# argumentcomputer/lurk-beta

Hardware: AMD Instinct MI355X
Metric: MSM Mscalar-mul/s (Pallas Pedersen commitment, bases+scalars resident in HBM) (higher is better)
Workload: dtype u32x8 (255-bit Montgomery, integer VALU)

## Files before the change

lurk_beta_amd/csrc/curve29.cuh:

```cuda
#pragma once
#include "curve.cuh"
#include "field29.cuh"

#ifndef LURK_ACC_Y3_ROW
#define LURK_ACC_Y3_ROW 1
#endif
#ifndef LURK_ACC_AFFINE_FIRST
#define LURK_ACC_AFFINE_FIRST 1
#endif
#ifndef LURK_F29_RARE_ATTR
#define LURK_F29_RARE_ATTR __attribute__((noinline))
#endif

namespace lurk {

template <class P>
LURK_HD F29<P> f29_carry_signed(const int32_t* t) {
    F29<P> r;
    int32_t c = 0;
#pragma unroll
    for (int i = 0; i < 8; i++) {
        int32_t x = t[i] + c;
        r.l[i] = (uint32_t)x & F29_MASK;
        c = x >> 29;
    }
    r.l[8] = (uint32_t)(t[8] + c);
    return r;
}


template <class P>
LURK_HD F29<P> f29_reduce_pasta(const F29<P>& v) {
    const uint32_t k = v.l[8] >> 22;
    const uint32_t km1 = k ? k - 1 : 0;
    int32_t t[9];
    uint64_t c = 0;
#pragma unroll
    for (int i = 0; i < 5; i++) {
        c += (uint64_t)km1 * f29_mod<P>(i);
        t[i] = (int32_t)v.l[i] - (int32_t)((uint32_t)c & F29_MASK);
        c >>= 29;
    }
    t[5] = (int32_t)v.l[5] - (int32_t)(uint32_t)c;
    t[6] = (int32_t)v.l[6];
    t[7] = (int32_t)v.l[7];
    t[8] = (int32_t)(v.l[8] & ((1u << 22) - 1u)) + (k ? (int32_t)(1u << 22) : 0);
    return f29_carry_signed<P>(t);
}
template <class P>
LURK_HD F29<P> f29_reduce_general(const F29<P>& v) {
    constexpr uint32_t D = (P::mod(7) >> 8) + 1u;
    static_assert(D > (1u << 21) && D <= (1u << 22), "f29_reduce_general: the modulus must have 253 or 254 bits");
    constexpr uint64_t mu = ((uint64_t)1 << 53) / D;
    F29_ASSERT(v.l[8] < (1u << 31), "f29_reduce: top limb >= 2^31");
    const uint32_t q = (uint32_t)(((uint64_t)v.l[8] * mu) >> 53);
    int32_t t[9];
    uint64_t c = 0;
#pragma unroll
    for (int i = 0; i < 8; i++) {
        c += (uint64_t)q * f29_mod<P>(i);
        t[i] = (int32_t)v.l[i] - (int32_t)((uint32_t)c & F29_MASK);
        c >>= 29;
    }
    c += (uint64_t)q * f29_mod<P>(8);
    t[8] = (int32_t)v.l[8] - (int32_t)(uint32_t)c;
    const F29<P> r = f29_carry_signed<P>(t);
    F29_ASSERT(r.l[8] < (1u << 24), "f29_reduce: result not below 2^256");
    return r;
}
template <class P>
LURK_HD F29<P> f29_reduce(const F29<P>& v) {
    if constexpr (f29_pasta_shape<P>()) return f29_reduce_pasta<P>(v);
    else return f29_reduce_general<P>(v);
}

template <class P>
struct Xyzz29 {
    F29<P> x, y, zz, zzz;
};

template <class P>
LURK_HD Xyzz<P> xyzz29_to_xyzz(const Xyzz29<P>& a, bool is_identity) {
    if (is_identity) return xyzz_identity<P>();
    Xyzz<P> r;
    r.x = f29_to_mont256<P>(a.x);
    r.y = f29_to_mont256<P>(a.y);
    r.zz = f29_to_mont256<P>(a.zz);
    r.zzz = f29_to_mont256<P>(a.zzz);
    return r;
}
template <class P>
LURK_HD void xyzz29_from_xyzz(const Xyzz<P>& a, Xyzz29<P>& r, bool& is_identity) {
    is_identity = xyzz_is_identity<P>(a);
    r.x = f29_from_mont256<P>(a.x);
    r.y = f29_from_mont256<P>(a.y);
    r.zz = f29_from_mont256<P>(a.zz);
    r.zzz = f29_from_mont256<P>(a.zzz);
}

template <class P>
LURK_HD uint32_t f29_multiple_candidate(const F29<P>& v) {
    if constexpr (f29_pasta_shape<P>()) return v.l[0];
    else return (v.l[0] * ((0u - f29_inv<P>()) & F29_MASK)) & F29_MASK;
}
template <class P>
LURK_HD bool f29_maybe_multiple_of_p(const F29<P>& v) {
    return f29_multiple_candidate<P>(v) < (f29_pasta_shape<P>() ? 128u : 256u);
}
template <class P>
LURK_HD bool f29_is_multiple_of_p(const F29<P>& v) {
    const uint32_t k = f29_multiple_candidate<P>(v);
    uint64_t c = 0;
    bool eq = true;
#pragma unroll
    for (int i = 0; i < 8; i++) {
        c += (uint64_t)k * f29_mod<P>(i);
        eq = eq && (v.l[i] == ((uint32_t)c & F29_MASK));
        c >>= 29;
    }
    c += (uint64_t)k * f29_mod<P>(8);
    return eq && (uint64_t)v.l[8] == c;
}

template <class P>
LURK_HD LURK_F29_RARE_ATTR Xyzz29<P> xyzz29_double_affine(F29<P> qx, F29<P> qy_signed) {
    const F29<P> u = f29_dbl<P>(qy_signed);
    const F29<P> v = f29_mul<P>(u, u);
    const F29<P> w = f29_mul30<P>(u, v);
    const F29<P> s = f29_mul30<P>(qx, v);
    const F29<P> xx = f29_sqr30<P>(qx);
    const F29<P> m = f29_carry<P>(f29_add<P>(f29_dbl<P>(xx), xx));
    const F29<P> m2 = f29_sqr30<P>(m);
    Xyzz29<P> r;
    r.x = f29_reduce<P>(f29_carry<P>(f29_sub<P>(m2, f29_dbl<P>(s))));
    const F29<P> t1 = f29_mul<P>(m, f29_sub<P>(s, r.x));
    const F29<P> t2 = f29_mul30<P>(w, qy_signed);
    r.y = f29_reduce<P>(f29_carry<P>(f29_sub<P>(t1, t2)));
    r.zz = v;
    r.zzz = w;
    return r;
}

template <class P, bool ACC_AFFINE = false>
LURK_HD void xyzz29_madd(Xyzz29<P>& acc, bool& acc_id, const Affine<P>& q, bool negate) {
    if (affine_is_identity<P>(q)) return;
    const F29<P> qx = f29_from_mont256<P>(q.x);
    const F29<P> qy = f29_from_mont256<P>(q.y);
    if (acc_id) {
        acc.x = qx;
        acc.y = negate ? f29_reduce<P>(f29_carry<P>(f29_sub<P>(f29_zero<P>(), qy))) : qy;
        Fe<P> one = fe_one<P>();
        acc.zz = f29_from_mont256<P>(one);
        acc.zzz = acc.zz;
        acc_id = false;
        return;
    }
    F29_ASSERT_LIMBS(acc.x, 29, "acc.x"); F29_ASSERT_TOP(acc.x, 27, "acc.x");
    F29_ASSERT_LIMBS(acc.y, 29, "acc.y"); F29_ASSERT_TOP(acc.y, 27, "acc.y");
    F29_ASSERT_LIMBS(acc.zz, 29, "acc.zz"); F29_ASSERT_TOP(acc.zz, 27, "acc.zz");
    F29_ASSERT_LIMBS(acc.zzz, 29, "acc.zzz"); F29_ASSERT_TOP(acc.zzz, 27, "acc.zzz");
    const F29<P> u2 = ACC_AFFINE ? qx : f29_mul30<P>(qx, acc.zz);
    const F29<P> s2 = ACC_AFFINE ? qy : f29_mul30<P>(qy, acc.zzz);
    const F29<P> p = f29_carry<P>(f29_sub<P>(u2, acc.x));
    F29<P> r;
#pragma unroll
    for (int i = 0; i < 9; i++) {
        F29_ASSERT(f29_bias<P>(i) >= acc.y.l[i], "madd: Y1 limb above the bias");
        r.l[i] = s2.l[i] + (negate ? acc.y.l[i] : f29_bias<P>(i) - acc.y.l[i]);
    }
    r = f29_carry<P>(r);
    if (f29_maybe_multiple_of_p<P>(p) && f29_is_multiple_of_p<P>(p)) {
        if (f29_maybe_multiple_of_p<P>(r) && f29_is_multiple_of_p<P>(r)) {
            const F29<P> qys = negate ? f29_reduce<P>(f29_carry<P>(f29_sub<P>(f29_zero<P>(), qy))) : qy;
            acc = xyzz29_double_affine<P>(qx, qys);
        } else {
            acc_id = true;
        }
        return;
    }
    const F29<P> pp = f29_sqr30<P>(p);
    const F29<P> ppp = f29_mul30<P>(p, pp);
    const F29<P> qq = f29_mul30<P>(acc.x, pp);
    const F29<P> r2 = f29_sqr30<P>(r);
    F29<P> x3 = f29_sub<P>(f29_sub<P>(r2, ppp), f29_dbl<P>(qq));
    x3 = f29_reduce<P>(f29_carry<P>(x3));
    F29<P> d;
#pragma unroll
    for (int i = 0; i < 9; i++) {
        F29_ASSERT(f29_bias<P>(i) >= qq.l[i] && f29_bias<P>(i) >= x3.l[i], "madd: Q / X3 limb above the bias");
        d.l[i] = negate ? x3.l[i] + (f29_bias<P>(i) - qq.l[i]) : qq.l[i] + (f29_bias<P>(i) - x3.l[i]);
    }
#if LURK_ACC_Y3_ROW
    Dot29<P> row;
    dot29_init<P>(row);
    dot29_mac<P>(row, r, f29_carry<P>(d));
    dot29_mac<P>(row, f29_carry<P>(f29_sub<P>(f29_zero<P>(), acc.y)), ppp);
    F29<P> y3 = f29_reduce<P>(dot29_finish2<P>(row));
#else
    const F29<P> t1 = f29_mul<P>(r, d);
    const F29<P> t2 = f29_mul30<P>(acc.y, ppp);
    F29<P> y3 = f29_reduce<P>(f29_carry<P>(f29_sub<P>(t1, t2)));
#endif
    acc.x = x3;
    acc.y = y3;
    if (ACC_AFFINE) {
        acc.zz = f29_reduce<P>(pp);
        acc.zzz = f29_reduce<P>(ppp);
    } else {
        acc.zz = f29_mul30<P>(acc.zz, pp);
        acc.zzz = f29_mul30<P>(acc.zzz, ppp);
    }
}

template <class P>
LURK_HD Xyzz29<P> xyzz29_dbl(const Xyzz29<P>& a) {
    const F29<P> u = f29_dbl<P>(a.y);
    const F29<P> v = f29_mul<P>(u, u);
    const F29<P> w = f29_mul30<P>(u, v);
    const F29<P> s = f29_mul30<P>(a.x, v);
    const F29<P> xx = f29_sqr30<P>(a.x);
    const F29<P> m = f29_carry<P>(f29_add<P>(f29_dbl<P>(xx), xx));
    const F29<P> m2 = f29_sqr30<P>(m);
    Xyzz29<P> r;
    r.x = f29_reduce<P>(f29_carry<P>(f29_sub<P>(m2, f29_dbl<P>(s))));
    const F29<P> t1 = f29_mul<P>(m, f29_sub<P>(s, r.x));
    const F29<P> t2 = f29_mul30<P>(w, a.y);
    r.y = f29_reduce<P>(f29_carry<P>(f29_sub<P>(t1, t2)));
    r.zz = f29_mul30<P>(v, a.zz);
    r.zzz = f29_mul30<P>(w, a.zzz);
    return r;
}

template <class P>
LURK_HD LURK_F29_RARE_ATTR Xyzz29<P> xyzz29_double_general(Xyzz29<P> a) {
    const Xyzz<P> d = xyzz_dbl<P>(xyzz29_to_xyzz<P>(a, false));
    Xyzz29<P> r;
    bool id;
    xyzz29_from_xyzz<P>(d, r, id);
    return r;
}

template <class P>
LURK_HD void xyzz29_add(Xyzz29<P>& acc, bool& acc_id, const Xyzz29<P>& q, bool q_id) {
    if (q_id) return;
    if (acc_id) {
        acc = q;
        acc_id = false;
        return;
    }
    F29_ASSERT_LIMBS(acc.x, 29, "add acc.x"); F29_ASSERT_TOP(acc.x, 27, "add acc.x");
    F29_ASSERT_LIMBS(acc.y, 29, "add acc.y"); F29_ASSERT_TOP(acc.y, 27, "add acc.y");
    F29_ASSERT_LIMBS(acc.zz, 29, "add acc.zz"); F29_ASSERT_TOP(acc.zz, 27, "add acc.zz");
    F29_ASSERT_LIMBS(acc.zzz, 29, "add acc.zzz"); F29_ASSERT_TOP(acc.zzz, 27, "add acc.zzz");
    F29_ASSERT_LIMBS(q.x, 29, "add q.x"); F29_ASSERT_TOP(q.x, 27, "add q.x");
    F29_ASSERT_LIMBS(q.y, 29, "add q.y"); F29_ASSERT_TOP(q.y, 27, "add q.y");
    F29_ASSERT_LIMBS(q.zz, 29, "add q.zz"); F29_ASSERT_TOP(q.zz, 27, "add q.zz");
    F29_ASSERT_LIMBS(q.zzz, 29, "add q.zzz"); F29_ASSERT_TOP(q.zzz, 27, "add q.zzz");
    const F29<P> u1 = f29_mul30<P>(acc.x, q.zz);
    const F29<P> u2 = f29_mul30<P>(q.x, acc.zz);
    const F29<P> s1 = f29_mul30<P>(acc.y, q.zzz);
    const F29<P> s2 = f29_mul30<P>(q.y, acc.zzz);
    const F29<P> p = f29_carry<P>(f29_sub<P>(u2, u1));
    const F29<P> r = f29_carry<P>(f29_sub<P>(s2, s1));
    if (f29_maybe_multiple_of_p<P>(p) && f29_is_multiple_of_p<P>(p)) {
        if (f29_maybe_multiple_of_p<P>(r) && f29_is_multiple_of_p<P>(r)) acc = xyzz29_double_general<P>(acc);
        else acc_id = true;
        return;
    }
    const F29<P> pp = f29_sqr30<P>(p);
    const F29<P> ppp = f29_mul30<P>(p, pp);
    const F29<P> qq = f29_mul30<P>(u1, pp);
    const F29<P> r2 = f29_sqr30<P>(r);
    F29<P> x3 = f29_sub<P>(f29_sub<P>(r2, ppp), f29_dbl<P>(qq));
    x3 = f29_reduce<P>(f29_carry<P>(x3));
    F29<P> d;
#pragma unroll
    for (int i = 0; i < 9; i++) {
        F29_ASSERT(f29_bias<P>(i) >= x3.l[i], "add: X3 limb above the bias");
        d.l[i] = qq.l[i] + (f29_bias<P>(i) - x3.l[i]);
    }
    Dot29<P> row;
    dot29_init<P>(row);
    dot29_mac<P>(row, r, f29_carry<P>(d));
    dot29_mac<P>(row, f29_carry<P>(f29_sub<P>(f29_zero<P>(), s1)), ppp);
    const F29<P> y3 = f29_reduce<P>(dot29_finish2<P>(row));
    const F29<P> zz12 = f29_mul30<P>(acc.zz, q.zz);
    const F29<P> zzz12 = f29_mul30<P>(acc.zzz, q.zzz);
    acc.x = x3;
    acc.y = y3;
    acc.zz = f29_mul30<P>(zz12, pp);
    acc.zzz = f29_mul30<P>(zzz12, ppp);
}

template <class P>
LURK_HD Xyzz<P> xyzz_sum_via29(const Xyzz<P>* pts, uint32_t nt) {
    if (nt == 0) return xyzz_identity<P>();
    if (nt == 1) return pts[0];
    Xyzz29<P> acc, q;
    bool acc_id, q_id;
    xyzz29_from_xyzz<P>(pts[0], acc, acc_id);
    for (uint32_t i = 1; i < nt; i++) {
        xyzz29_from_xyzz<P>(pts[i], q, q_id);
        xyzz29_add<P>(acc, acc_id, q, q_id);
    }
    return xyzz29_to_xyzz<P>(acc, acc_id);
}

typedef uint32_t Rec16 __attribute__((vector_size(16), may_alias));
struct Rec64 {
    Rec16 q[4];
};
template <class P>
LURK_HD Rec64 rec64_load(const Affine<P>* table, uint32_t e) {
    static_assert(sizeof(Affine<P>) == 64 && alignof(Affine<P>) >= 16, "a table record is four aligned 16-byte words");
    const Rec16* p = reinterpret_cast<const Rec16*>(table + (e & 0x7fffffffu));
    Rec64 r;
#pragma unroll
    for (int i = 0; i < 4; i++) r.q[i] = p[i];
    return r;
}
template <class P>
LURK_HD Affine<P> rec64_affine(const Rec64& r) {
    Affine<P> a;
#pragma unroll
    for (int i = 0; i < 8; i++) {
        a.x.l[i] = r.q[i >> 2][i & 3];
        a.y.l[i] = r.q[2 + (i >> 2)][i & 3];
    }
    return a;
}
template <class P>
LURK_HD Affine<P> msm_task_next29(const uint32_t* sorted, const Affine<P>* table, uint32_t j, uint32_t last, bool& neg_next, uint32_t& e_ahead,
                                  Rec64& rec, bool& negate) {
    const Affine<P> q = rec64_affine<P>(rec);
    negate = neg_next;
    neg_next = (e_ahead & 0x80000000u) != 0;
    rec = rec64_load<P>(table, e_ahead);
    e_ahead = sorted[j + 2 < last ? j + 2 : j];
    return q;
}

template <class P, bool PIPELINED = false>
LURK_HD void msm_task_accumulate29_raw(const uint32_t* sorted, uint32_t first, uint32_t last, const Affine<P>* table, Xyzz29<P>& acc, bool& acc_id) {
    acc.x = acc.y = acc.zz = acc.zzz = f29_zero<P>();
    acc_id = true;
    if (PIPELINED) {
        if (first >= last) return;
        const uint32_t e_first = sorted[first];
        bool neg_next = (e_first & 0x80000000u) != 0;
        Rec64 rec = rec64_load<P>(table, e_first);
        uint32_t e_ahead = sorted[first + 1 < last ? first + 1 : first];
        uint32_t j = first;
        bool negate;
#if LURK_ACC_AFFINE_FIRST
        {
            const Affine<P> q = msm_task_next29<P>(sorted, table, j, last, neg_next, e_ahead, rec, negate);
            xyzz29_madd<P>(acc, acc_id, q, negate);
            j++;
        }
        if (j < last) {
            const Affine<P> q = msm_task_next29<P>(sorted, table, j, last, neg_next, e_ahead, rec, negate);
            if (!acc_id) xyzz29_madd<P, true>(acc, acc_id, q, negate);
            else xyzz29_madd<P>(acc, acc_id, q, negate);
            j++;
        }
#endif
        for (; j < last; j++) {
            const Affine<P> q = msm_task_next29<P>(sorted, table, j, last, neg_next, e_ahead, rec, negate);
            xyzz29_madd<P>(acc, acc_id, q, negate);
        }
        return;
    }
#if LURK_ACC_AFFINE_FIRST
    uint32_t j = first;
    if (j < last) {
        const uint32_t e = sorted[j++];
        xyzz29_madd<P>(acc, acc_id, table[e & 0x7fffffffu], (e & 0x80000000u) != 0);
    }
    if (j < last) {
        const uint32_t e = sorted[j++];
        const Affine<P> q = table[e & 0x7fffffffu];
#if LURK_ACC_AFFINE_FIRST
        if (!acc_id) xyzz29_madd<P, true>(acc, acc_id, q, (e & 0x80000000u) != 0);
        else
#endif
            xyzz29_madd<P>(acc, acc_id, q, (e & 0x80000000u) != 0);
    }
    for (; j < last; j++) {
        const uint32_t e = sorted[j];
        const Affine<P> q = table[e & 0x7fffffffu];
        xyzz29_madd<P>(acc, acc_id, q, (e & 0x80000000u) != 0);
    }
#else
    for (uint32_t j = first; j < last; j++) {
        const uint32_t e = sorted[j];
#ifdef LURK_ACC_DEBUG_TABLE_MASK
        const Affine<P> q = table[e & LURK_ACC_DEBUG_TABLE_MASK];
#else
        const Affine<P> q = table[e & 0x7fffffffu];
#endif
        xyzz29_madd<P>(acc, acc_id, q, (e & 0x80000000u) != 0);
    }
#endif
}
template <class P, bool PIPELINED = false>
LURK_HD Xyzz<P> msm_task_accumulate29(const uint32_t* sorted, uint32_t first, uint32_t last, const Affine<P>* table) {
    Xyzz29<P> acc;
    bool acc_id;
    msm_task_accumulate29_raw<P, PIPELINED>(sorted, first, last, table, acc, acc_id);
    return xyzz29_to_xyzz<P>(acc, acc_id);
}

}
```

lurk_beta_amd/csrc/msm.hip:

```cpp
#include "common.hpp"
#include "dispatch.hpp"
#include "msm_core.cuh"
#include "msm_ctx.hpp"
#include "msm_launch_plan.hpp"
#include "msm_sort.hpp"
#include "msm_stages.hpp"

namespace lurk {

struct MsmLaunch {
    MsmLaunchPlan plan;
    int sel = -1;
    hipEvent_t gate = nullptr;
    hipStream_t acc_stream = nullptr;
    const std::function<void()>* before_accumulate = nullptr;
};

template <class P, class SF>
struct MsmCtx : MsmCtxBase {
    DevBuf own_bases;
    DevBuf pre_scratch;
    const Affine<P>* table = nullptr;
    DevBuf small_table;

    struct Work {
        std::mutex mu;
        DevBuf inter, sorted, block_hist, part_cnt, part_start, cnt, bucket_start, task_start, group_tasks, group_task_base, task_info,
            task_order, len_hist, partials, buckets, big_list, big_count, planes_a, planes_b, canon, small_counter;
        Xyzz<P>* host_pts = nullptr;
        size_t ws_n = 0, ws_entries = 0, ws_nt = 0;
        uint32_t ws_NB = 0;
        hipStream_t stream = nullptr;
        hipStream_t acc_stream = nullptr;
        hipEvent_t ready = nullptr, planned = nullptr, accumulated = nullptr;
        DevBuf cursor;
        bool placement_valid = false;
        int sel = -1;
        bool small_ready = false;
        hipStream_t pending_stream = nullptr;
        bool pending = false;
        size_t pending_n = 0;
        ~Work() {
            if (host_pts) (void)hipHostFree(host_pts);
            if (stream) (void)hipStreamDestroy(stream);
            if (acc_stream) (void)hipStreamDestroy(acc_stream);
            if (ready) (void)hipEventDestroy(ready);
            if (planned) (void)hipEventDestroy(planned);
            if (accumulated) (void)hipEventDestroy(accumulated);
        }
    };
    static size_t small_form_bytes(size_t n) {
        const int cs = msm_small_window_bits(n);
        return msm_small_table_entries(n, cs) * sizeof(Affine<P>) + msm_small_scratch_bytes() + (size_t)msm_num_windows(cs) * n * 160;
    }
    struct WorkView {
        const Work& wk;
        static uint32_t* u32(const DevBuf& b) { return (uint32_t*)b.p; }
        uint32_t *sorted = u32(wk.sorted), *cnt = u32(wk.cnt), *bucket_start = u32(wk.bucket_start), *task_start = u32(wk.task_start),
                 *group_tasks = u32(wk.group_tasks), *group_task_base = u32(wk.group_task_base), *task_order = u32(wk.task_order),
                 *len_hist = u32(wk.len_hist), *big_list = u32(wk.big_list), *big_count = u32(wk.big_count), *cursor = u32(wk.cursor);
        uint2* task_info = (uint2*)wk.task_info.p;
        Xyzz<P>*partials = (Xyzz<P>*)wk.partials.p, *buckets = (Xyzz<P>*)wk.buckets.p;
        void *planes_a = wk.planes_a.p, *planes_b = wk.planes_b.p;
        MsmSortBufs sort_bufs() const {
            return MsmSortBufs{wk.inter.p, sorted, u32(wk.block_hist), u32(wk.part_cnt), u32(wk.part_start), cnt, bucket_start, wk.canon.p,
                               {big_count, len_hist, cursor}, {1, 2 * (MSM_S + 1), MSM_PLACEMENT_BASE + 512}};
        }
    };
    Work work[MSM_SLOTS];
    std::mutex fg_mu;
    Work* last_fg = nullptr;
    std::mutex acc_ring_mu;
    Work* acc_ring[MSM_SLOTS] = {};
    int acc_ring_pos = 0, acc_ring_count = 0;

    MsmShape shape(size_t n, int sel = -1) const { return msm_make_shape(c, precomputed, npoints, n, sel); }

    void set_bases_device(const void* d_bases, size_t n, bool copy, bool precompute, int c_override, hipStream_t s, int small_pref = 0) {
        npoints = n;
        precomputed = precompute;
        small = false;
        small_table.release();
        bool small_form = precompute && !c_override && n > 0 && n <= MSM_SMALL_MAX_POINTS && small_pref >= 0;
        LURK_REQUIRE(small_pref <= 0 || small_form, "LURK_MSM_FLAG_SMALL_FORM: the small form needs the precompute flag, no window override and 1 .. 2^16 points");
        const size_t need = small_form ? small_form_bytes(n) : 0;
        if (small_form && small_pref > 0) {
            size_t free_b = 0, total_b = 0;
            LURK_HIP_CHECK(hipMemGetInfo(&free_b, &total_b));
            const char* cap_env = getenv("LURK_MSM_SMALL_FORM_MAX_MB");
            const size_t cap_mb = cap_env ? (size_t)atoll(cap_env) : (size_t)0;
            if (need > free_b || (cap_mb && need > (cap_mb << 20)))
                throw HipFailure{LURK_HIP_ERR_OOM, "LURK_MSM_FLAG_SMALL_FORM: the small-commitment form of this key needs " + std::to_string(need >> 20) +
                                                       " MiB (free: " + std::to_string(free_b >> 20) + " MiB" + (cap_mb ? ", LURK_MSM_SMALL_FORM_MAX_MB=" + std::to_string(cap_mb) : std::string()) + ")"};
        }
        if (small_form && small_pref == 0) {
            size_t free_b = 0, total_b = 0;
            LURK_HIP_CHECK(hipMemGetInfo(&free_b, &total_b));
            if (need > free_b / 4) small_form = false;
        }
        if (small_form) {
            c = msm_small_window_bits(n);
            const int Ws = msm_num_windows(c);
            own_bases.alloc(n * sizeof(Affine<P>));
            LURK_HIP_CHECK(hipMemcpyAsync(own_bases.p, d_bases, n * sizeof(Affine<P>), hipMemcpyDeviceToDevice, s));
            table = own_bases.as<Affine<P>>();
            {
                DevBuf wbases((size_t)Ws * n * sizeof(Affine<P>)), scratch(msm_precompute_scratch_bytes(n, Ws));
                {
                    ProfScope ps("msm_precompute", s);
                    msm_launch_precompute<P>((const Affine<P>*)d_bases, n, wbases.as<Affine<P>>(), c, Ws, scratch.p, s);
                }
                small_table.alloc(msm_small_table_entries(n, c) * sizeof(Affine<P>));
                msm_small_build_table<P>(wbases.as<Affine<P>>(), n, c, small_table.as<Affine<P>>(), s);
            }
            small = true;
            return;
        }
        c = precompute ? (n <= ((size_t)1 << 18) ? 16 : 20) : MSM_C_PLAIN;
        if (c_override) c = c_override;
        LURK_REQUIRE(c >= 16 && c <= 20, "window bits must be in 16..20");
        LURK_REQUIRE(precompute || c == MSM_C_PLAIN, "the plain mode uses 16-bit windows");
        const int W = msm_num_windows(c);
        LURK_REQUIRE((size_t)W * n < ((size_t)1 << 31), "too many points: windows x points must stay below 2^31");
        if (precompute) {
            if (keep_buffers) own_bases.ensure((size_t)W * n * sizeof(Affine<P>));
            else own_bases.alloc((size_t)W * n * sizeof(Affine<P>));
            if (n) {
                DevBuf once;
                DevBuf& scratch = keep_buffers ? pre_scratch : once;
                scratch.ensure(msm_precompute_scratch_bytes(n, W));
                {
                    ProfScope ps("msm_precompute", s);
                    msm_launch_precompute<P>((const Affine<P>*)d_bases, n, own_bases.as<Affine<P>>(), c, W, scratch.p, s);
                }
                LURK_HIP_CHECK(hipStreamSynchronize(s));
            }
            LURK_HIP_CHECK(hipStreamSynchronize(s));
            table = own_bases.as<Affine<P>>();
        } else if (copy) {
            own_bases.alloc(n * sizeof(Affine<P>));
            LURK_HIP_CHECK(hipMemcpyAsync(own_bases.p, d_bases, n * sizeof(Affine<P>), hipMemcpyDeviceToDevice, s));
            LURK_HIP_CHECK(hipStreamSynchronize(s));
            table = own_bases.as<Affine<P>>();
        } else {
            table = (const Affine<P>*)d_bases;
        }
    }

    DevBuf oneshot_scalars;
    static constexpr size_t ONESHOT_SAMPLES = 4096;
    const void* oneshot_host = nullptr;
    size_t oneshot_n = 0;
    std::vector<char> oneshot_samples;
    static size_t oneshot_sample_pos(size_t k, size_t n) { return (size_t)(((unsigned __int128)k * n) / ONESHOT_SAMPLES); }
    bool oneshot_key_matches(const void* bases, size_t n) const {
        if (!oneshot_host || bases != oneshot_host || n > oneshot_n || oneshot_samples.empty()) return false;
        const size_t cnt = oneshot_n < ONESHOT_SAMPLES ? oneshot_n : ONESHOT_SAMPLES;
        for (size_t k = 0; k < cnt; k++) {
            const size_t i = oneshot_n < ONESHOT_SAMPLES ? k : oneshot_sample_pos(k, oneshot_n);
            if (i >= n) break;
            if (memcmp((const char*)bases + i * 64, oneshot_samples.data() + k * 64, 64) != 0) return false;
        }
        return true;
    }
    void oneshot_key_remember(const void* bases, size_t n) {
        const size_t cnt = n < ONESHOT_SAMPLES ? n : ONESHOT_SAMPLES;
        oneshot_samples.resize(cnt * 64);
        for (size_t k = 0; k < cnt; k++) memcpy(oneshot_samples.data() + k * 64, (const char*)bases + (n < ONESHOT_SAMPLES ? k : oneshot_sample_pos(k, n)) * 64, 64);
        oneshot_host = bases;
        oneshot_n = n;
    }
    void run_oneshot(const void* bases, const void* scalars, size_t n, int is_mont, void* out) override {
        if (n == 0) {
            put_identity(out);
            return;
        }
        LURK_REQUIRE((size_t)msm_num_windows(MSM_C_PLAIN) * n < ((size_t)1 << 31), "too many points");
        Work& wk = work[0];
        std::lock_guard<std::mutex> lk(wk.mu);
        LURK_REQUIRE(!wk.pending, "slot 0 has a submitted commitment that was not waited for");
        const bool cache_on = oneshot_key_cache_enabled(), cached = cache_on && oneshot_key_matches(bases, n);
        if (!cached) {
            oneshot_host = nullptr;
            own_bases.ensure(n * sizeof(Affine<P>));
        }
        oneshot_scalars.ensure(n * 32);
        table = own_bases.as<Affine<P>>();
        npoints = n;
        precomputed = false;
        small = false;
        small_table.release();
        c = MSM_C_PLAIN;
        ensure_streams(wk);
        hipStream_t s = wk.stream;
        LURK_HIP_CHECK(hipMemcpyAsync(oneshot_scalars.p, scalars, n * 32, hipMemcpyHostToDevice, s));
        const std::function<void()> upload_bases = [&] {
            if (!cached) LURK_HIP_CHECK(hipMemcpyAsync(own_bases.p, bases, n * sizeof(Affine<P>), hipMemcpyHostToDevice, s));
        };
        MsmLaunch L = launch_for(MsmSubmitClass::SYNC, n);
        L.before_accumulate = &upload_bases;
        enqueue(wk, oneshot_scalars.p, n, is_mont, s, L);
        LURK_HIP_CHECK(hipStreamSynchronize(s));
        if (!cached && cache_on) oneshot_key_remember(bases, n);
        host_tail(wk, n, out);
    }
    void rebind(const void* d_bases, size_t n) override {
        LURK_REQUIRE((size_t)msm_num_windows(MSM_C_PLAIN) * n < ((size_t)1 << 31), "too many points");
        for (auto& wk : work) {
            std::lock_guard<std::mutex> lk(wk.mu);
            LURK_REQUIRE(!wk.pending, "a slot has a commitment in flight");
        }
        own_bases.release();
        small_table.release();
        small = false;
        table = (const Affine<P>*)d_bases;
        npoints = n;
        precomputed = false;
        c = MSM_C_PLAIN;
    }
    void reserve(size_t n, int slots) override {
        LURK_REQUIRE(n <= npoints, "more scalars than bases in the context");
        LURK_REQUIRE(slots >= 1 && slots <= MSM_SLOTS, "slot count out of range");
        if (n == 0) return;
        if (small) {
            DevBuf zeros(32);
            LURK_HIP_CHECK(hipMemset(zeros.p, 0, 32));
            LURK_HIP_CHECK(hipStreamSynchronize(nullptr));
            for (int k = 0; k < slots; k++) {
                Work& wk = work[k];
                std::lock_guard<std::mutex> lk(wk.mu);
                LURK_REQUIRE(!wk.pending, "slot is busy");
                ensure_streams(wk);
                enqueue(wk, zeros.p, 1, 0, wk.stream, launch_for(MsmSubmitClass::SYNC, 1));
                LURK_HIP_CHECK(hipStreamSynchronize(wk.stream));
            }
            return;
        }
        const MsmShape sh = shape(n);
        const size_t nz = n < 256 ? n : 256;
        DevBuf zeros(nz * 32);
        LURK_HIP_CHECK(hipMemset(zeros.p, 0, nz * 32));
        LURK_HIP_CHECK(hipStreamSynchronize(nullptr));
        for (int k = 0; k < slots; k++) {
            Work& wk = work[k];
            std::lock_guard<std::mutex> lk(wk.mu);
            LURK_REQUIRE(!wk.pending, "slot is busy");
            ensure_workspace(wk, sh);
            ensure_streams(wk);
            enqueue(wk, zeros.p, nz, 0, wk.stream, launch_for(MsmSubmitClass::SYNC, nz));
            LURK_HIP_CHECK(hipStreamSynchronize(wk.stream));
        }
    }
    const void* device_table() const override { return table; }
    void adopt_table(DevBuf&& buf, size_t n, bool precomputed_, int c_) override {
        own_bases = std::move(buf);
        table = own_bases.as<Affine<P>>();
        small_table.release();
        small = false;
        npoints = n;
        precomputed = precomputed_;
        c = c_;
    }

    void ensure_workspace_small(Work& wk, hipStream_t s) {
        if (wk.small_ready) return;
        wk.partials.ensure(msm_small_group_bytes());
        wk.small_counter.ensure(16);
        LURK_HIP_CHECK(hipMemsetAsync(wk.small_counter.p, 0, 16, s));
        if (!wk.host_pts) LURK_HIP_CHECK(hipHostMalloc((void**)&wk.host_pts, (size_t)MSM_MAX_W * 20 * sizeof(Xyzz<P>)));
        wk.small_ready = true;
    }

    size_t ntask_max(const MsmShape& sh) const { return (size_t)sh.NB + (size_t)sh.W * sh.n / sh.S + 1; }

    void ensure_workspace(Work& wk, const MsmShape& sh) {
        const size_t entries = (size_t)sh.W * sh.n, nt = ntask_max(sh);
        if (wk.ws_n != 0 && entries <= wk.ws_entries && nt <= wk.ws_nt && sh.NB <= wk.ws_NB) return;
        wk.inter.ensure(msm_inter_bytes(entries));
        wk.sorted.ensure(entries * 4);
        wk.block_hist.ensure((size_t)MSM_NB1 * MSM_P_MAX * 4);
        wk.part_cnt.ensure(MSM_P_MAX * 4);
        wk.part_start.ensure((MSM_P_MAX + 1) * 4);
        wk.cnt.ensure((size_t)sh.NB * 4);
        wk.bucket_start.ensure((size_t)sh.NB * 4);
        wk.task_start.ensure((size_t)sh.NG * (MSM_GRP + 1) * 4);
        wk.group_tasks.ensure(64 * 4);
        wk.group_task_base.ensure(64 * 4);
        wk.task_info.ensure(nt * sizeof(uint2));
        wk.task_order.ensure(nt * 4);
        wk.len_hist.ensure(2 * (MSM_S + 1) * 4);
        wk.partials.ensure(nt * sizeof(Xyzz<P>));
        wk.buckets.ensure((size_t)sh.NB * sizeof(Xyzz<P>));
        wk.big_list.ensure((size_t)sh.NB * 4);
        wk.big_count.ensure(16);
        wk.cursor.ensure(4 * (MSM_PLACEMENT_BASE + 512));
        wk.planes_a.ensure(msm_reduce_plane_bytes(sh.NB));
        wk.planes_b.ensure(msm_reduce_plane_bytes(sh.NB));
        if (!wk.host_pts) LURK_HIP_CHECK(hipHostMalloc((void**)&wk.host_pts, (size_t)MSM_MAX_W * 20 * sizeof(Xyzz<P>)));
        wk.ws_n = sh.n > wk.ws_n ? sh.n : wk.ws_n;
        wk.ws_entries = entries > wk.ws_entries ? entries : wk.ws_entries;
        wk.ws_nt = nt > wk.ws_nt ? nt : wk.ws_nt;
        wk.ws_NB = sh.NB > wk.ws_NB ? sh.NB : wk.ws_NB;
    }

    MsmLaunch launch_for(MsmSubmitClass cls, size_t n, int sel = -1) const {
        MsmLaunch L;
        L.sel = sel;
        size_t entries = 0;
        uint32_t NB = 0;
        if (!small) {
            const MsmShape sh = shape(n, sel);
            entries = (size_t)sh.W * sh.n;
            NB = sh.NB;
        }
        L.plan = msm_launch_plan(cls, entries, NB, msm_tuning(), msm_follow_wgs());
        return L;
    }

    void enqueue(Work& wk, const void* d_scalars, size_t n, int is_mont, hipStream_t s, const MsmLaunch& L) {
        if (small) {
            ensure_workspace_small(wk, s);
            msm_small_launch<P, SF>(d_scalars, n, is_mont, small_table.as<Affine<P>>(), c, wk.partials.p, wk.small_counter.template as<uint32_t>(), wk.host_pts, s);
            if (wk.planned) LURK_HIP_CHECK(hipEventRecord(wk.planned, s));
            return;
        }
        const MsmAccForm form = L.plan.form;
        const bool direct = form == MsmAccForm::DIRECT;
        MsmShape sh = shape(n, L.sel);
        const int low = L.plan.low_prio ? 1 : 0;
        sh.low_prio = low;
        ensure_workspace(wk, sh);
        if (is_mont) wk.canon.ensure(n * 32);
        const WorkView v{wk};
        const size_t nt = ntask_max(sh);
        {
            ProfScope ps("msm_sort", s);
            msm_launch_sort<SF>(sh, d_scalars, is_mont, v.sort_bufs(), s);
        }
        if (!direct) {
            ProfScope ps("msm_tasks", s);
            msm_launch_plan_tasks(v.cnt, v.bucket_start, v.task_start, v.group_tasks, v.group_task_base, sh.NG, v.task_info, v.len_hist, v.task_order, nt,
                                  (uint32_t)sh.S, low, s);
        }
        if (L.before_accumulate) (*L.before_accumulate)();
        if (wk.planned) LURK_HIP_CHECK(hipEventRecord(wk.planned, s));
        if (L.gate && !direct) LURK_HIP_CHECK(hipStreamWaitEvent(s, L.gate, 0));
        switch (form) {
        case MsmAccForm::DIRECT: {
            ProfScope ps("msm_accumulate_direct", s);
            msm_launch_bucket_direct<P>(v.sorted, table, v.bucket_start, v.cnt, sh.NB, (size_t)sh.W * sh.n, v.buckets, v.big_list, v.big_count, s);
            break;
        }
        case MsmAccForm::PERSISTENT_SLOT_STREAM: {
            wk.placement_valid = true;
            {
                ProfScope ps("msm_accumulate_persistent", s);
                msm_launch_accumulate_persistent<P>(v.sorted, table, v.task_info, v.task_order, v.group_task_base, sh.NG, v.partials, v.cursor, s, L.plan.wgs_per_cu);
            }
            LURK_HIP_CHECK(hipEventRecord(wk.accumulated, s));
            break;
        }
        case MsmAccForm::PERSISTENT_ACC_STREAM: {
            wk.placement_valid = true;
            LURK_HIP_CHECK(hipStreamWaitEvent(L.acc_stream, wk.planned, 0));
            if (msm_tuning().max_acc >= 1) {
                const int max_acc = msm_tuning().max_acc;
                std::lock_guard<std::mutex> lk(acc_ring_mu);
                if (acc_ring_count >= max_acc) {
                    Work* gate = acc_ring[(acc_ring_pos + MSM_SLOTS - max_acc) % MSM_SLOTS];
                    if (gate && gate != &wk && gate->accumulated) LURK_HIP_CHECK(hipStreamWaitEvent(L.acc_stream, gate->accumulated, 0));
                }
                acc_ring[acc_ring_pos % MSM_SLOTS] = &wk;
                acc_ring_pos++;
                if (acc_ring_count < MSM_SLOTS) acc_ring_count++;
            }
            {
                ProfScope ps("msm_accumulate_persistent", L.acc_stream);
                msm_launch_accumulate_persistent<P>(v.sorted, table, v.task_info, v.task_order, v.group_task_base, sh.NG, v.partials, v.cursor, L.acc_stream);
            }
            LURK_HIP_CHECK(hipEventRecord(wk.accumulated, L.acc_stream));
            LURK_HIP_CHECK(hipStreamWaitEvent(s, wk.accumulated, 0));
            break;
        }
        case MsmAccForm::PLAIN: {
            {
                ProfScope ps("msm_accumulate", s);
                msm_launch_accumulate<P>(v.sorted, table, v.task_info, v.task_order, v.group_task_base, sh.NG, v.partials, nt, s);
            }
            if (wk.accumulated) LURK_HIP_CHECK(hipEventRecord(wk.accumulated, s));
            break;
        }
        }
        if (!direct) {
            ProfScope ps("msm_finalize", s);
            msm_launch_finalize<P>(v.partials, v.cnt, v.task_start, v.group_task_base, sh.NB, v.buckets, v.big_list, v.big_count, (uint32_t)sh.S, s);
            msm_launch_big_buckets<P>(v.partials, v.cnt, v.task_start, v.group_task_base, v.buckets, v.big_list, v.big_count, (uint32_t)sh.S, s);
        }
        {
            ProfScope ps("msm_reduce", s);
            msm_launch_reduce<P>(v.buckets, v.planes_a, v.planes_b, sh.c, sh.G, sh.B, wk.host_pts, s);
        }
        LURK_HIP_CHECK(hipGetLastError());
    }

    static void put_point(void* out, const Jacobian<P>& j) { memcpy(out, &j, sizeof(j)); }
    static void put_identity(void* out) { put_point(out, jacobian_from_affine<P>(Affine<P>{fe_zero<P>(), fe_zero<P>()})); }
    void host_tail(Work& wk, size_t n, void* out) {
        if (small) {
            const unsigned K = msm_small_out_points(msm_small_groups(n, c));
            Xyzz<P> total = xyzz_identity<P>();
            for (unsigned k = 0; k < K; k++) xyzz_add<P>(total, wk.host_pts[k]);
            put_point(out, jacobian_from_affine<P>(xyzz_to_affine<P>(total)));
            return;
        }
        const MsmShape sh = shape(n);
        const Xyzz<P> total = msm_planes_horner_windows<P>(wk.host_pts, sh.G, sh.c);
        put_point(out, jacobian_from_affine<P>(xyzz_to_affine<P>(total)));
    }
    void run(const void* d_scalars, size_t n, int is_mont, hipStream_t s, void* out_jac96_host) override {
        LURK_REQUIRE(n <= npoints, "more scalars than bases in the context");
        void* out = out_jac96_host;
        if (n == 0) {
            put_identity(out);
            return;
        }
        Work& wk = work[0];
        std::lock_guard<std::mutex> lk(wk.mu);
        LURK_REQUIRE(!wk.pending, "slot 0 has a submitted commitment that was not waited for");
        enqueue(wk, d_scalars, n, is_mont, s, launch_for(MsmSubmitClass::SYNC, n));
        LURK_HIP_CHECK(hipStreamSynchronize(s));
        host_tail(wk, n, out);
    }

    void submit_pair(int slot, const void* d_scalars, size_t n, int is_mont, hipStream_t after, int sel_bit) override {
        LURK_REQUIRE(precomputed && !small, "a pair of commitments in one pass needs the window-table form of a key (precompute flag, more than 2^16 points "
                                            "or a window-bit override)");
        LURK_REQUIRE(sel_bit >= 0 && sel_bit < 31, "selector bit out of range");
        LURK_REQUIRE(n > 0, "empty pair");
        submit_impl(slot, d_scalars, n, is_mont, after, LURK_MSM_SUBMIT_FOREGROUND, sel_bit);
    }
    void wait_pair(int slot, void* out_lo, void* out_hi, bool xyzz) override {
        LURK_REQUIRE(slot >= 0 && slot < MSM_SLOTS, "slot out of range");
        Work& wk = work[slot];
        std::lock_guard<std::mutex> lk(wk.mu);
        LURK_REQUIRE(wk.pending && wk.sel >= 0, "no pair was submitted on this slot");
        wk.pending = false;
        LURK_HIP_CHECK(hipStreamSynchronize(wk.pending_stream ? wk.pending_stream : wk.stream));
        void* outs[2] = {out_lo, out_hi};
        for (int g = 0; g < 2; g++) {
            const Xyzz<P> t = msm_planes_horner_windows<P>(wk.host_pts + (size_t)g * c, 1, c);
            if (xyzz) memcpy(outs[g], &t, sizeof(t));
            else put_point(outs[g], jacobian_from_affine<P>(xyzz_to_affine<P>(t)));
        }
        wk.sel = -1;
    }
    void submit(int slot, const void* d_scalars, size_t n, int is_mont, hipStream_t after, int mode) override {
        submit_impl(slot, d_scalars, n, is_mont, after, mode, -1);
    }
    void submit_impl(int slot, const void* d_scalars, size_t n, int is_mont, hipStream_t after, int mode, int sel_bit) {
        LURK_REQUIRE(slot >= 0 && slot < MSM_SLOTS, "slot out of range");
        LURK_REQUIRE(n <= npoints, "more scalars than bases in the context");
        Work& wk = work[slot];
        std::lock_guard<std::mutex> lk(wk.mu);
        LURK_REQUIRE(!wk.pending, "slot is busy: wait for it first");
        wk.sel = sel_bit;
        ensure_streams(wk);
        if (n) {
            const MsmSubmitClass cls = (MsmSubmitClass)mode;
            MsmLaunch L = launch_for(cls, n, sel_bit);
            wk.pending_stream = wk.stream;
            LURK_HIP_CHECK(hipEventRecord(wk.ready, after));
            LURK_HIP_CHECK(hipStreamWaitEvent(wk.pending_stream, wk.ready, 0));
            {
                std::lock_guard<std::mutex> lk2(fg_mu);
                if (cls == MsmSubmitClass::BACKGROUND && last_fg && last_fg != &wk && last_fg->planned)
                    LURK_HIP_CHECK(hipStreamWaitEvent(wk.pending_stream, last_fg->planned, 0));
                if (cls == MsmSubmitClass::FOLLOW && last_fg && last_fg != &wk && last_fg->accumulated) L.gate = last_fg->accumulated;
                if (cls == MsmSubmitClass::FOREGROUND) last_fg = &wk;
            }
            if (L.plan.uses_acc_stream) L.acc_stream = ensure_acc_stream(wk);
            enqueue(wk, d_scalars, n, is_mont, wk.pending_stream, L);
        }
        wk.pending = true;
        wk.pending_n = n;
    }

    hipStream_t ensure_acc_stream(Work& wk) {
        if (!wk.acc_stream) {
            int least = 0, greatest = 0;
            LURK_HIP_CHECK(hipDeviceGetStreamPriorityRange(&least, &greatest));
            LURK_HIP_CHECK(hipStreamCreateWithPriority(&wk.acc_stream, hipStreamNonBlocking, least));
        }
        return wk.acc_stream;
    }

    void ensure_streams(Work& wk) {
        if (!wk.stream) {
            int least = 0, greatest = 0;
            LURK_HIP_CHECK(hipDeviceGetStreamPriorityRange(&least, &greatest));
            LURK_HIP_CHECK(hipStreamCreateWithPriority(&wk.stream, hipStreamNonBlocking, greatest));
            LURK_HIP_CHECK(hipEventCreateWithFlags(&wk.ready, hipEventDisableTiming));
            LURK_HIP_CHECK(hipEventCreateWithFlags(&wk.planned, hipEventDisableTiming));
            LURK_HIP_CHECK(hipEventCreateWithFlags(&wk.accumulated, hipEventDisableTiming));
        }
    }

    void wait(int slot, void* out_jac96_host) override {
        LURK_REQUIRE(slot >= 0 && slot < MSM_SLOTS, "slot out of range");
        Work& wk = work[slot];
        std::lock_guard<std::mutex> lk(wk.mu);
        LURK_REQUIRE(wk.pending, "nothing was submitted on this slot");
        LURK_REQUIRE(wk.sel < 0, "a pair is pending on this slot: use lurk_hip_msm_ctx_wait_pair");
        void* out = out_jac96_host;
        wk.pending = false;
        if (wk.pending_n == 0) {
            put_identity(out);
            return;
        }
        LURK_HIP_CHECK(hipStreamSynchronize(wk.pending_stream ? wk.pending_stream : wk.stream));
        if (wk.placement_valid && msm_tuning().placement_log) log_placement(wk);
        host_tail(wk, wk.pending_n, out);
    }
    void log_placement(Work& wk) {
        std::vector<uint32_t> h(MSM_PLACEMENT_BASE + 512);
        LURK_HIP_CHECK(hipMemcpy(h.data(), wk.cursor.p, h.size() * 4, hipMemcpyDeviceToHost));
        int hist[8] = {0}, used = 0;
        for (int i = 0; i < 512; i++) {
            uint32_t c = h[MSM_PLACEMENT_BASE + i];
            if (c) used++;
            hist[c > 7 ? 7 : c]++;
        }
        fprintf(stderr, "[lurk_hip] accumulate placement: %d CUs used; CUs with 1/2/3/4+ workgroups: %d/%d/%d/%d\n", used, hist[1], hist[2], hist[3],
                hist[4] + hist[5] + hist[6] + hist[7]);
        wk.placement_valid = false;
    }
};

MsmCtxBase* new_ctx(int curve) {
    MsmCtxBase* c = nullptr;
    with_curve(curve, [&](auto P, auto SF) { c = new MsmCtx<decltype(P), decltype(SF)>(); });
    c->curve = curve;
    c->device = current_device();
    return c;
}
void ctx_set_bases(MsmCtxBase* c, const void* d_bases, size_t n, bool copy, int flags, hipStream_t s) {
    bool pre = (flags & LURK_MSM_FLAG_PRECOMPUTE) != 0;
    int c_override = (flags >> 8) & 0xff;
    LURK_REQUIRE(!((flags & LURK_MSM_FLAG_SMALL_FORM) && (flags & LURK_MSM_FLAG_NO_SMALL_FORM)), "LURK_MSM_FLAG_SMALL_FORM and LURK_MSM_FLAG_NO_SMALL_FORM exclude each other");
    const int small_pref = (flags & LURK_MSM_FLAG_SMALL_FORM) ? 1 : (flags & LURK_MSM_FLAG_NO_SMALL_FORM) ? -1 : 0;
    with_curve(c->curve, [&](auto P, auto SF) {
        static_cast<MsmCtx<decltype(P), decltype(SF)>*>(c)->set_bases_device(d_bases, n, copy, pre, c_override, s, small_pref);
    });
}

}
```

lurk_beta_amd/csrc/msm_acc.hip:

```cpp
#ifndef LURK_ACC_RADIX29
#define LURK_ACC_RADIX29 1
#endif
#if !LURK_ACC_RADIX29
#define LURK_MUL_FORCE_INLINE
#endif
#include "common.hpp"
#include "msm_acc_task.cuh"

namespace lurk {

template <class P>
__global__ __launch_bounds__(MSM_ACC_BLOCK) void msm_accumulate_kernel(const uint32_t* __restrict__ sorted, const Affine<P>* __restrict__ table,
                                                                         const uint2* __restrict__ task_info, const uint32_t* __restrict__ order,
                                                                         const uint32_t* __restrict__ group_task_base, int NG,
                                                                         Xyzz<P>* __restrict__ partials) {
#if !defined(LURK_ACC_NO_SETPRIO)
    __builtin_amdgcn_s_setprio(1);
#endif
    uint32_t i = blockIdx.x * MSM_ACC_BLOCK + threadIdx.x;
    if (i >= group_task_base[NG]) return;
    msm_accumulate_task<P>(i, sorted, table, task_info, order, partials);
}

template <class P>
void msm_launch_accumulate(const uint32_t* sorted, const Affine<P>* table, const uint2* task_info, const uint32_t* order,
                           const uint32_t* group_task_base, int NG, Xyzz<P>* partials, size_t nt, hipStream_t s) {
    hipLaunchKernelGGL((msm_accumulate_kernel<P>), dim3(div_up(nt, MSM_ACC_BLOCK)), dim3(MSM_ACC_BLOCK), 0, s, sorted, table, task_info, order,
                       group_task_base, NG, partials);
}
#define LURK_ACC_INSTANTIATE(P)                                                                                                             \
    template void msm_launch_accumulate<P>(const uint32_t*, const Affine<P>*, const uint2*, const uint32_t*, const uint32_t*, int, Xyzz<P>*, \
                                           size_t, hipStream_t);
#ifdef LURK_MSM_BN254_TU
LURK_ACC_INSTANTIATE(Bn254Fq)
LURK_ACC_INSTANTIATE(Bn254Fr)
#else
LURK_ACC_INSTANTIATE(PallasFp)
LURK_ACC_INSTANTIATE(PallasFq)
#endif

}
```

lurk_beta_amd/csrc/msm_acc_persistent.hip:

```cpp
#ifndef LURK_ACC_RADIX29
#define LURK_ACC_RADIX29 1
#endif
#if !LURK_ACC_RADIX29
#define LURK_MUL_FORCE_INLINE
#endif
#include "common.hpp"
#include "msm_acc_task.cuh"

namespace lurk {

__device__ __forceinline__ uint32_t msm_cu_index() {
    const uint32_t hw = __builtin_amdgcn_s_getreg((4 ) | (0 << 6) | (31 << 11));
    const uint32_t xcc = __builtin_amdgcn_s_getreg((20 ) | (0 << 6) | (3 << 11));
    return (xcc & 7u) * 64u + ((hw >> 13) & 3u) * 16u + ((hw >> 8) & 15u);
}

template <class P, bool PIPELINED>
#ifndef LURK_PERSIST_MIN_BLOCKS
#define LURK_PERSIST_MIN_BLOCKS 1
#endif
#define LURK_PERSIST_VGPR_BUDGET 192
__global__ __launch_bounds__(MSM_ACC_BLOCK, LURK_PERSIST_MIN_BLOCKS) __attribute__((amdgpu_num_vgpr(LURK_PERSIST_VGPR_BUDGET / 2))) void msm_accumulate_persistent_kernel(const uint32_t* __restrict__ sorted, const Affine<P>* __restrict__ table,
                                                                                    const uint2* __restrict__ task_info,
                                                                                    const uint32_t* __restrict__ order,
                                                                                    const uint32_t* __restrict__ group_task_base, int NG,
                                                                                    Xyzz<P>* __restrict__ partials, uint32_t* __restrict__ cursor) {
    const uint32_t ntasks = group_task_base[NG];
    const uint32_t lane = threadIdx.x & 63u;
    if (threadIdx.x == 0) atomicAdd(&cursor[MSM_PLACEMENT_BASE + msm_cu_index()], 1u);
    for (;;) {
        uint32_t base = 0;
        if (lane == 0) base = atomicAdd(cursor, 64u);
        base = __builtin_amdgcn_readfirstlane(base);
        if (base >= ntasks) break;
        if (base + lane < ntasks) msm_accumulate_task<P, PIPELINED>(base + lane, sorted, table, task_info, order, partials);
    }
}

template <class P>
void msm_launch_accumulate_persistent(const uint32_t* sorted, const Affine<P>* table, const uint2* task_info, const uint32_t* order,
                                      const uint32_t* group_task_base, int NG, Xyzz<P>* partials, uint32_t* cursor, hipStream_t s, unsigned wgs_per_cu) {
    static const unsigned wgs = [] { const char* e = getenv("LURK_MSM_PERSIST_WGS"); int v = e ? atoi(e) : 1; return (unsigned)(v < 1 ? 1 : v > 4 ? 4 : v); }();
    const unsigned waves = wgs_per_cu ? wgs_per_cu : wgs;
    if (waves == 1)
        hipLaunchKernelGGL((msm_accumulate_persistent_kernel<P, true>), dim3((unsigned)num_cus()), dim3(MSM_ACC_BLOCK), 0, s, sorted, table, task_info, order,
                           group_task_base, NG, partials, cursor);
    else
        hipLaunchKernelGGL((msm_accumulate_persistent_kernel<P, false>), dim3((unsigned)num_cus() * waves), dim3(MSM_ACC_BLOCK), 0, s, sorted, table, task_info, order,
                           group_task_base, NG, partials, cursor);
}
#define LURK_ACC_PERSISTENT_INSTANTIATE(P)                                                                                                    \
    template void msm_launch_accumulate_persistent<P>(const uint32_t*, const Affine<P>*, const uint2*, const uint32_t*, const uint32_t*, int, \
                                                      Xyzz<P>*, uint32_t*, hipStream_t, unsigned);
#ifdef LURK_MSM_BN254_TU
LURK_ACC_PERSISTENT_INSTANTIATE(Bn254Fq)
LURK_ACC_PERSISTENT_INSTANTIATE(Bn254Fr)
#else
LURK_ACC_PERSISTENT_INSTANTIATE(PallasFp)
LURK_ACC_PERSISTENT_INSTANTIATE(PallasFq)
#endif

}
```

lurk_beta_amd/csrc/msm_acc_task.cuh:

```cuda
#pragma once
#include "msm_core.cuh"
#include "curve29.cuh"
#include "msm_stages.hpp"

namespace lurk {

#ifndef LURK_ACC_TASK_NOINLINE
#define LURK_ACC_TASK_NOINLINE 0
#endif
#if LURK_ACC_TASK_NOINLINE
#define LURK_ACC_TASK_ATTR __attribute__((noinline))
#else
#define LURK_ACC_TASK_ATTR __forceinline__
#endif
template <class P, bool PIPELINED = false>
__device__ LURK_ACC_TASK_ATTR void msm_accumulate_task(uint32_t i, const uint32_t* __restrict__ sorted, const Affine<P>* __restrict__ table,
                                                    const uint2* __restrict__ task_info, const uint32_t* __restrict__ order,
                                                    Xyzz<P>* __restrict__ partials) {
    uint32_t t = order[i];
    uint2 ti = task_info[t];
#if LURK_ACC_RADIX29
    partials[t] = msm_task_accumulate29<P, PIPELINED>(sorted, ti.x, ti.y, table);
#else
    partials[t] = msm_task_accumulate<P>(sorted, ti.x, ti.y, table);
#endif
}

}
```

lurk_beta_amd/csrc/msm_bucket_direct.hip:

```cpp
#include "common.hpp"
#include "msm_core.cuh"
#include "curve29.cuh"
#include "msm_stages.hpp"

namespace lurk {

constexpr int DIRECT_BLOCK = 256;
constexpr uint32_t DIRECT_CAP = 64;

template <class P, int L>
__global__ __launch_bounds__(DIRECT_BLOCK) void msm_bucket_direct_kernel(const uint32_t* __restrict__ sorted, const Affine<P>* __restrict__ table,
                                                                           const uint32_t* __restrict__ bucket_start, const uint32_t* __restrict__ cnt,
                                                                           uint32_t NB, Xyzz<P>* __restrict__ buckets, uint32_t* __restrict__ big_list,
                                                                           uint32_t* __restrict__ big_count) {
    __builtin_amdgcn_s_setprio(1);
    const size_t lane = (size_t)blockIdx.x * DIRECT_BLOCK + threadIdx.x;
    size_t key = lane / L;
    const uint32_t sub = (uint32_t)(lane % L);
    const bool live = key < NB;
    if (!live) key = NB - 1;
    uint32_t n = live ? cnt[key] : 0u;
    const uint32_t start = bucket_start[key];
    const bool big = n > (uint32_t)L * DIRECT_CAP;
    if (big) {
        if (sub == 0) big_list[atomicAdd(big_count, 1u)] = (uint32_t)key;
        n = 0;
    }
    const uint32_t per = (n + L - 1) / L;
    uint32_t first = start + sub * per, last = first + per;
    if (first > start + n) first = start + n;
    if (last > start + n) last = start + n;
    Xyzz29<P> acc;
    bool acc_id;
    msm_task_accumulate29_raw<P>(sorted, first, last, table, acc, acc_id);
#pragma unroll
    for (int off = L / 2; off >= 1; off >>= 1) {
        Xyzz29<P> o;
        bool o_id;
#pragma unroll
        for (int k = 0; k < 9; k++) {
            o.x.l[k] = __shfl_xor(acc.x.l[k], off);
            o.y.l[k] = __shfl_xor(acc.y.l[k], off);
            o.zz.l[k] = __shfl_xor(acc.zz.l[k], off);
            o.zzz.l[k] = __shfl_xor(acc.zzz.l[k], off);
        }
        o_id = __shfl_xor((int)acc_id, off) != 0;
        xyzz29_add<P>(acc, acc_id, o, o_id);
    }
    if (live && !big && sub == 0) buckets[key] = xyzz29_to_xyzz<P>(acc, acc_id);
}

template <class P>
__global__ __launch_bounds__(DIRECT_BLOCK) void msm_bucket_direct_big_kernel(const uint32_t* __restrict__ sorted, const Affine<P>* __restrict__ table,
                                                                               const uint32_t* __restrict__ bucket_start, const uint32_t* __restrict__ cnt,
                                                                               Xyzz<P>* __restrict__ buckets, const uint32_t* __restrict__ big_list,
                                                                               const uint32_t* __restrict__ big_count) {
    __builtin_amdgcn_s_setprio(1);
    extern __shared__ uint4 lds_raw[];
    Xyzz<P>* sh = reinterpret_cast<Xyzz<P>*>(lds_raw);
    const uint32_t nbig = *big_count;
    for (uint32_t i = blockIdx.x; i < nbig; i += gridDim.x) {
        const uint32_t key = big_list[i], n = cnt[key], start = bucket_start[key];
        Xyzz29<P> a29;
        a29.x = a29.y = a29.zz = a29.zzz = f29_zero<P>();
        bool a_id = true;
        for (uint32_t j = threadIdx.x; j < n; j += DIRECT_BLOCK) {
            const uint32_t e = sorted[start + j];
            xyzz29_madd<P>(a29, a_id, table[e & 0x7fffffffu], (e & 0x80000000u) != 0);
        }
        Xyzz<P> acc = xyzz29_to_xyzz<P>(a29, a_id);
        const int t = threadIdx.x;
        sh[t] = acc;
        __syncthreads();
        for (int stride = DIRECT_BLOCK / 2; stride >= 1; stride >>= 1) {
            if (t < stride) {
                xyzz_add<P>(acc, sh[t + stride]);
                sh[t] = acc;
            }
            __syncthreads();
        }
        if (t == 0) buckets[key] = acc;
        __syncthreads();
    }
}

#ifndef LURK_MSM_BN254_TU
int msm_bucket_direct_lanes(size_t NB, size_t entries) {
    int L = 1;
    while (L < 4 && NB * (size_t)(2 * L) <= 131072 && entries / (NB * (size_t)(2 * L)) >= 4) L *= 2;
    return L;
}
#endif

template <class P>
void msm_launch_bucket_direct(const uint32_t* sorted, const Affine<P>* table, const uint32_t* bucket_start, const uint32_t* cnt, uint32_t NB, size_t entries,
                              Xyzz<P>* buckets, uint32_t* big_list, uint32_t* big_count, hipStream_t s) {
    const int L = msm_bucket_direct_lanes(NB, entries);
    const dim3 grid((unsigned)div_up((size_t)NB * L, DIRECT_BLOCK)), block(DIRECT_BLOCK);
    if (L == 1) hipLaunchKernelGGL((msm_bucket_direct_kernel<P, 1>), grid, block, 0, s, sorted, table, bucket_start, cnt, NB, buckets, big_list, big_count);
    else if (L == 2) hipLaunchKernelGGL((msm_bucket_direct_kernel<P, 2>), grid, block, 0, s, sorted, table, bucket_start, cnt, NB, buckets, big_list, big_count);
    else hipLaunchKernelGGL((msm_bucket_direct_kernel<P, 4>), grid, block, 0, s, sorted, table, bucket_start, cnt, NB, buckets, big_list, big_count);
    hipLaunchKernelGGL((msm_bucket_direct_big_kernel<P>), dim3(128), block, DIRECT_BLOCK * sizeof(Xyzz<P>), s, sorted, table, bucket_start, cnt, buckets, big_list,
                       big_count);
}
#define LURK_DIRECT_INSTANTIATE(P)                                                                                                                      \
    template void msm_launch_bucket_direct<P>(const uint32_t*, const Affine<P>*, const uint32_t*, const uint32_t*, uint32_t, size_t, Xyzz<P>*, uint32_t*, \
                                              uint32_t*, hipStream_t);
#ifdef LURK_MSM_BN254_TU
LURK_DIRECT_INSTANTIATE(Bn254Fq)
LURK_DIRECT_INSTANTIATE(Bn254Fr)
#else
LURK_DIRECT_INSTANTIATE(PallasFp)
LURK_DIRECT_INSTANTIATE(PallasFq)
#endif

}
```

lurk_beta_amd/csrc/msm_finalize.hip:

```cpp
#include "common.hpp"
#include "msm_core.cuh"
#include "curve29.cuh"
#include "msm_stages.hpp"

namespace lurk {

#ifndef LURK_FINALIZE_WAVES
#define LURK_FINALIZE_WAVES 4
#endif
#define LURK_FINALIZE_BOUNDS __launch_bounds__(256, LURK_FINALIZE_WAVES)
template <class P>
__global__ LURK_FINALIZE_BOUNDS void msm_finalize_kernel(const Xyzz<P>* __restrict__ partials, const uint32_t* __restrict__ cnt,
                                                             const uint32_t* __restrict__ task_start,
                                                             const uint32_t* __restrict__ group_task_base, uint32_t NB,
                                                             Xyzz<P>* __restrict__ buckets, uint32_t* __restrict__ big_list,
                                                             uint32_t* __restrict__ big_count, uint32_t S) {
    __builtin_amdgcn_s_setprio(3);
    const size_t key = (size_t)blockIdx.x * 256 + threadIdx.x;
    if (key >= NB) return;
    const uint32_t g = (uint32_t)(key / MSM_GRP), b = (uint32_t)(key % MSM_GRP);
    const uint32_t nt = (cnt[key] + S - 1) / S;
    const uint32_t first = group_task_base[g] + task_start[(size_t)g * (MSM_GRP + 1) + b];
    if (nt > MSM_FIN_SMALL) {
        big_list[atomicAdd(big_count, 1u)] = (uint32_t)key;
        return;
    }
    buckets[key] = xyzz_sum_via29<P>(partials + first, nt);
}

template <class P>
void msm_launch_finalize(const Xyzz<P>* partials, const uint32_t* cnt, const uint32_t* task_start, const uint32_t* group_task_base, uint32_t NB,
                         Xyzz<P>* buckets, uint32_t* big_list, uint32_t* big_count, uint32_t S, hipStream_t s) {
    hipLaunchKernelGGL((msm_finalize_kernel<P>), dim3(div_up((size_t)NB, 256)), dim3(256), 0, s, partials, cnt, task_start, group_task_base, NB, buckets,
                       big_list, big_count, S);
}
#define LURK_FINALIZE_INSTANTIATE(P)                                                                                                          \
    template void msm_launch_finalize<P>(const Xyzz<P>*, const uint32_t*, const uint32_t*, const uint32_t*, uint32_t, Xyzz<P>*, uint32_t*, uint32_t*, \
                                         uint32_t, hipStream_t);
#ifdef LURK_MSM_BN254_TU
LURK_FINALIZE_INSTANTIATE(Bn254Fq)
LURK_FINALIZE_INSTANTIATE(Bn254Fr)
#else
LURK_FINALIZE_INSTANTIATE(PallasFp)
LURK_FINALIZE_INSTANTIATE(PallasFq)
#endif

}
```

lurk_beta_amd/csrc/msm_launch_plan.hpp:

```cpp
#pragma once
#include <cstddef>
#include <cstdint>
#include <cstdlib>

#include "../../include/lurk_hip.h"

namespace lurk {

enum class MsmSubmitClass {
    SYNC = -1,
    DEFAULT = LURK_MSM_SUBMIT_DEFAULT,
    FOREGROUND = LURK_MSM_SUBMIT_FOREGROUND,
    BACKGROUND = LURK_MSM_SUBMIT_BACKGROUND,
    FOLLOW = LURK_MSM_SUBMIT_FOLLOW,
};

enum class MsmAccForm {
    DIRECT,
    PLAIN,
    PERSISTENT_ACC_STREAM,
    PERSISTENT_SLOT_STREAM,
};

struct MsmTuning {
    int persistent = 1, max_acc = 2, placement_log = 0, bucket_direct = 1;
    size_t persistent_min = (size_t)24 << 20;
    static MsmTuning from_env() {
        auto geti = [](const char* k, int d) { const char* v = getenv(k); return v ? atoi(v) : d; };
        MsmTuning t;
        t.persistent = geti("LURK_MSM_ACC_PERSISTENT", 1);
        t.persistent_min = (size_t)geti("LURK_MSM_PERSISTENT_MIN_MENTRIES", 24) << 20;
        t.max_acc = geti("LURK_MSM_MAX_ACC", 2);
        t.bucket_direct = geti("LURK_MSM_BUCKET_DIRECT", 1);
        t.placement_log = geti("LURK_MSM_PLACEMENT_LOG", 0);
        if (t.max_acc > 2) t.max_acc = 0;
        return t;
    }
};
inline const MsmTuning& msm_tuning() {
    static const MsmTuning t = MsmTuning::from_env();
    return t;
}
inline int msm_follow_wgs() {
    static const int wgs = [] { const char* v = getenv("LURK_MSM_FOLLOW_WGS"); const int x = v ? atoi(v) : 2; return x < 0 ? 0 : x > 3 ? 3 : x; }();
    return wgs;
}

constexpr uint32_t MSM_DIRECT_MAX_BUCKETS = 131072;
constexpr size_t MSM_DIRECT_MAX_ENTRIES = (size_t)1 << 21;

struct MsmLaunchPlan {
    MsmAccForm form;
    bool low_prio;
    unsigned wgs_per_cu;
    bool uses_acc_stream;
};

inline MsmLaunchPlan msm_launch_plan(MsmSubmitClass cls, size_t entries, uint32_t NB, const MsmTuning& tn, int follow_wgs) {
    const bool bg = cls == MsmSubmitClass::BACKGROUND, follow = cls == MsmSubmitClass::FOLLOW;
    const bool acc_stream = cls == MsmSubmitClass::DEFAULT || bg;
    MsmLaunchPlan pl{MsmAccForm::PLAIN, follow, 0u, acc_stream};
    if (tn.bucket_direct && !bg && !(acc_stream && tn.persistent == 2) && NB <= MSM_DIRECT_MAX_BUCKETS && entries <= MSM_DIRECT_MAX_ENTRIES) {
        pl.form = MsmAccForm::DIRECT;
    } else if (follow && follow_wgs > 0) {
        pl.form = MsmAccForm::PERSISTENT_SLOT_STREAM;
        pl.wgs_per_cu = (unsigned)follow_wgs;
    } else if (acc_stream && (bg || (tn.persistent == 1 ? entries >= tn.persistent_min : tn.persistent != 0))) {
        pl.form = MsmAccForm::PERSISTENT_ACC_STREAM;
    }
    return pl;
}

}
```

lurk_beta_amd/csrc/msm_plan.hip:

```cpp
#include "common.hpp"
#include "msm_core.cuh"
#include "msm_sort.hpp"
#include "msm_stages.hpp"

namespace lurk {

__device__ __forceinline__ void msm_set_wave_prio(int low) {
    if (low) __builtin_amdgcn_s_setprio(0);
    else __builtin_amdgcn_s_setprio(3);
}

__global__ __launch_bounds__(1024) void msm_taskscan_kernel(const uint32_t* __restrict__ cnt, uint32_t* __restrict__ task_start,
                                                              uint32_t* __restrict__ group_tasks, uint32_t S, int low) {
    msm_set_wave_prio(low);
    __shared__ uint32_t sh[1024];
    const int g = blockIdx.x, t = threadIdx.x;
    constexpr int PER = MSM_GRP / 1024;
    const uint4* src = reinterpret_cast<const uint4*>(cnt + (size_t)g * MSM_GRP + (size_t)t * PER);
    uint32_t c[PER];
    uint32_t tot = 0;
#pragma unroll
    for (int j = 0; j < PER / 4; j++) {
        uint4 v = src[j];
        c[4 * j] = (v.x + S - 1) / S;
        c[4 * j + 1] = (v.y + S - 1) / S;
        c[4 * j + 2] = (v.z + S - 1) / S;
        c[4 * j + 3] = (v.w + S - 1) / S;
        tot += c[4 * j] + c[4 * j + 1] + c[4 * j + 2] + c[4 * j + 3];
    }
    sh[t] = tot;
    __syncthreads();
    for (int off = 1; off < 1024; off <<= 1) {
        uint32_t a = t >= off ? sh[t - off] : 0;
        __syncthreads();
        sh[t] += a;
        __syncthreads();
    }
    uint32_t run = sh[t] - tot;
    uint32_t* dst = task_start + (size_t)g * (MSM_GRP + 1) + (size_t)t * PER;
#pragma unroll
    for (int j = 0; j < PER; j++) {
        dst[j] = run;
        run += c[j];
    }
    if (t == 1023) {
        task_start[(size_t)g * (MSM_GRP + 1) + MSM_GRP] = run;
        group_tasks[g] = run;
    }
}
constexpr int MSM_NG_MAX = 64;
__global__ __launch_bounds__(256) void msm_tasks_kernel(const uint32_t* __restrict__ cnt, const uint32_t* __restrict__ bucket_start,
                                                          const uint32_t* __restrict__ task_start, const uint32_t* __restrict__ group_tasks,
                                                          uint32_t* __restrict__ group_task_base_out, int NG, uint2* __restrict__ task_info, uint32_t S, int low) {
    msm_set_wave_prio(low);
    __shared__ uint32_t group_task_base[MSM_NG_MAX + 1];
    if (threadIdx.x == 0) {
        uint32_t run = 0;
        for (int g = 0; g < NG; g++) {
            group_task_base[g] = run;
            run += group_tasks[g];
        }
        group_task_base[NG] = run;
        if (blockIdx.x == 0)
            for (int g = 0; g <= NG; g++) group_task_base_out[g] = group_task_base[g];
    }
    __syncthreads();
    uint32_t t = blockIdx.x * 256 + threadIdx.x;
    if (t >= group_task_base[NG]) return;
    int g = 0;
    while (g + 1 < NG && group_task_base[g + 1] <= t) g++;
    uint32_t tl = t - group_task_base[g];
    const uint32_t* ts = task_start + (size_t)g * (MSM_GRP + 1);
    uint32_t b = msm_upper_slot(ts, MSM_GRP, tl);
    uint32_t part = tl - ts[b];
    size_t key = (size_t)g * MSM_GRP + b;
    uint32_t first = bucket_start[key] + part * S;
    uint32_t end = bucket_start[key] + cnt[key];
    task_info[t] = make_uint2(first, first + S < end ? first + S : end);
}

__global__ __launch_bounds__(1024) void msm_len_hist_kernel(const uint2* __restrict__ task_info, const uint32_t* __restrict__ group_task_base,
                                                              int NG, uint32_t* __restrict__ len_hist, uint32_t S, int low) {
    msm_set_wave_prio(low);
    __shared__ uint32_t sh[MSM_S + 1];
    if (threadIdx.x <= MSM_S) sh[threadIdx.x] = 0;
    __syncthreads();
    const uint32_t ntasks = group_task_base[NG];
    for (uint32_t base = blockIdx.x * 8192u; base < ntasks; base += gridDim.x * 8192u) {
        for (uint32_t k = 0; k < 8; k++) {
            uint32_t t = base + k * 1024u + threadIdx.x;
            uint32_t len = 0;
            if (t < ntasks) {
                uint2 ti = task_info[t];
                len = ti.y - ti.x;
            }
            unsigned long long full = __ballot(len == S);
            if (full && (threadIdx.x & 63) == (unsigned)(__ffsll((long long)full) - 1)) atomicAdd(&sh[S], (uint32_t)__popcll(full));
            if (len != 0 && len != S) atomicAdd(&sh[len], 1u);
        }
    }
    __syncthreads();
    if (threadIdx.x <= MSM_S && sh[threadIdx.x]) atomicAdd(&len_hist[threadIdx.x], sh[threadIdx.x]);
}
__global__ __launch_bounds__(1024) void msm_len_scatter_kernel(const uint2* __restrict__ task_info,
                                                                 const uint32_t* __restrict__ group_task_base, int NG,
                                                                 const uint32_t* __restrict__ len_hist, uint32_t* __restrict__ len_cursor,
                                                                 uint32_t* __restrict__ order, uint32_t S, int low) {
    msm_set_wave_prio(low);
    __shared__ uint32_t sh_cnt[MSM_S + 1], sh_base[MSM_S + 1], sh_class[MSM_S + 1];
    if (threadIdx.x == 0) {
        uint32_t run = 0;
        for (int l = (int)S; l >= 0; l--) {
            sh_class[l] = run;
            run += len_hist[l];
        }
    }
    __syncthreads();
    const uint32_t ntasks = group_task_base[NG];
    for (uint32_t base = blockIdx.x * 1024u; base < ntasks; base += gridDim.x * 1024u) {
        if (threadIdx.x <= MSM_S) sh_cnt[threadIdx.x] = 0;
        __syncthreads();
        uint32_t t = base + threadIdx.x;
        uint32_t len = 0, rank = 0;
        if (t < ntasks) {
            uint2 ti = task_info[t];
            len = ti.y - ti.x;
        }
        unsigned long long full = __ballot(len == S);
        if (len == S) {
            int lane = threadIdx.x & 63, leader = __ffsll((long long)full) - 1;
            uint32_t wbase = 0;
            if (lane == leader) wbase = atomicAdd(&sh_cnt[S], (uint32_t)__popcll(full));
            wbase = __shfl(wbase, leader);
            rank = wbase + (uint32_t)__popcll(full & ((1ull << lane) - 1ull));
        } else if (len != 0) {
            rank = atomicAdd(&sh_cnt[len], 1u);
        }
        __syncthreads();
        if (threadIdx.x <= MSM_S && sh_cnt[threadIdx.x]) sh_base[threadIdx.x] = sh_class[threadIdx.x] + atomicAdd(&len_cursor[threadIdx.x], sh_cnt[threadIdx.x]);
        __syncthreads();
        if (len != 0) order[sh_base[len] + rank] = t;
        __syncthreads();
    }
}

void msm_launch_plan_tasks(const uint32_t* cnt, const uint32_t* bucket_start, uint32_t* task_start, uint32_t* group_tasks, uint32_t* group_task_base,
                           int NG, uint2* task_info, uint32_t* len_hist, uint32_t* order, size_t nt, uint32_t S, int low, hipStream_t s) {
    hipLaunchKernelGGL(msm_taskscan_kernel, dim3(NG), dim3(1024), 0, s, cnt, task_start, group_tasks, S, low);
    hipLaunchKernelGGL(msm_tasks_kernel, dim3(div_up(nt, 256)), dim3(256), 0, s, cnt, bucket_start, task_start, group_tasks, group_task_base, NG, task_info, S,
                       low);
    hipLaunchKernelGGL(msm_len_hist_kernel, dim3(256), dim3(1024), 0, s, task_info, group_task_base, NG, len_hist, S, low);
    hipLaunchKernelGGL(msm_len_scatter_kernel, dim3(512), dim3(1024), 0, s, task_info, group_task_base, NG, len_hist, len_hist + MSM_S + 1, order, S, low);
}

template <class P, int BLOCK>
__device__ void block_tree_sum(Xyzz<P>& acc, Xyzz<P>* sh) {
    const int t = threadIdx.x;
    sh[t] = acc;
    __syncthreads();
    for (int stride = BLOCK / 2; stride >= 1; stride >>= 1) {
        if (t < stride) {
            xyzz_add<P>(acc, sh[t + stride]);
            sh[t] = acc;
        }
        __syncthreads();
    }
}

template <class P>
__global__ __launch_bounds__(256) void msm_big_bucket_kernel(const Xyzz<P>* __restrict__ partials, const uint32_t* __restrict__ cnt,
                                                               const uint32_t* __restrict__ task_start,
                                                               const uint32_t* __restrict__ group_task_base, Xyzz<P>* __restrict__ buckets,
                                                               const uint32_t* __restrict__ big_list, const uint32_t* __restrict__ big_count, uint32_t S) {
    msm_set_wave_prio(0);
    extern __shared__ uint4 lds_raw[];
    Xyzz<P>* sh = reinterpret_cast<Xyzz<P>*>(lds_raw);
    const uint32_t nbig = *big_count;
    for (uint32_t i = blockIdx.x; i < nbig; i += gridDim.x) {
        uint32_t key = big_list[i];
        uint32_t g = key / MSM_GRP, b = key % MSM_GRP;
        uint32_t nt = (cnt[key] + S - 1) / S;
        uint32_t first = group_task_base[g] + task_start[(size_t)g * (MSM_GRP + 1) + b];
        Xyzz<P> acc = xyzz_identity<P>();
        for (uint32_t j = threadIdx.x; j < nt; j += 256) xyzz_add<P>(acc, partials[first + j]);
        block_tree_sum<P, 256>(acc, sh);
        if (threadIdx.x == 0) buckets[key] = acc;
        __syncthreads();
    }
}

template <class P>
void msm_launch_big_buckets(const Xyzz<P>* partials, const uint32_t* cnt, const uint32_t* task_start, const uint32_t* group_task_base, Xyzz<P>* buckets,
                            const uint32_t* big_list, const uint32_t* big_count, uint32_t S, hipStream_t s) {
    hipLaunchKernelGGL((msm_big_bucket_kernel<P>), dim3(128), dim3(256), 256 * sizeof(Xyzz<P>), s, partials, cnt, task_start, group_task_base, buckets, big_list,
                       big_count, S);
}
#define LURK_BIG_BUCKETS_INSTANTIATE(P)                                                                                                                   \
    template void msm_launch_big_buckets<P>(const Xyzz<P>*, const uint32_t*, const uint32_t*, const uint32_t*, Xyzz<P>*, const uint32_t*, const uint32_t*, \
                                            uint32_t, hipStream_t);
LURK_BIG_BUCKETS_INSTANTIATE(PallasFp)
LURK_BIG_BUCKETS_INSTANTIATE(PallasFq)
LURK_BIG_BUCKETS_INSTANTIATE(Bn254Fq)
LURK_BIG_BUCKETS_INSTANTIATE(Bn254Fr)

}
```

lurk_beta_amd/csrc/msm_reduce.hip:

```cpp
#include "common.hpp"
#include "msm_core.cuh"
#include "curve29.cuh"

#ifdef LURK_REDUCE_VGPRS
#define LURK_REDUCE_BOUNDS __launch_bounds__(REDUCE_BLOCK, LURK_REDUCE_VGPRS)
#else
#define LURK_REDUCE_BOUNDS __launch_bounds__(REDUCE_BLOCK, 4)
#endif
#ifndef LURK_REDUCE_COMPACT
#define LURK_REDUCE_COMPACT 1
#endif

namespace lurk {

#if defined(LURK_REDUCE_NOADD)
template <class P>
__device__ __forceinline__ void level_add(Xyzz29<P>& r, bool& r_id, const Xyzz29<P>& h, bool h_id) {
#pragma unroll
    for (int i = 0; i < 9; i++) { r.x.l[i] ^= h.x.l[i]; r.y.l[i] ^= h.y.l[i]; r.zz.l[i] ^= h.zz.l[i]; r.zzz.l[i] ^= h.zzz.l[i]; }
    r_id = r_id && h_id;
}
#else
template <class P>
__device__ __forceinline__ void level_add(Xyzz29<P>& r, bool& r_id, const Xyzz29<P>& h, bool h_id) { xyzz29_add<P>(r, r_id, h, h_id); }
#endif

constexpr int REDUCE_BLOCK = 256;

template <class P>
struct Plane29 {
    Xyzz29<P> p;
    uint32_t id, pad[3];
};

template <class P>
__device__ __forceinline__ void plane_load(const Plane29<P>* __restrict__ src, Xyzz29<P>& v, bool& id) {
    const Plane29<P> r = *src;
    v = r.p;
    id = r.id != 0;
}

template <class P, bool FIRST, bool LAST>
__global__ LURK_REDUCE_BOUNDS void msm_planes29_kernel(const Xyzz<P>* __restrict__ buckets, const Plane29<P>* __restrict__ in,
                                                                      Plane29<P>* __restrict__ out, Xyzz<P>* __restrict__ out_host, int k, int G, uint32_t B) {
    __builtin_amdgcn_s_setprio(3);
    const size_t nseg_out = (size_t)B >> (k + 1);
    const size_t comps_out = (size_t)k + 2, comps_in = (size_t)k + 1;
    const size_t tid = (size_t)blockIdx.x * REDUCE_BLOCK + threadIdx.x;
    if (tid >= (size_t)G * nseg_out * comps_out) return;
#if LURK_REDUCE_COMPACT
    size_t comp, seg, g;
    const size_t adders = (size_t)G * nseg_out * comps_in;
    if (tid < adders) {
        comp = tid % comps_in;
        seg = (tid / comps_in) % nseg_out;
        g = tid / (comps_in * nseg_out);
    } else {
        comp = comps_in;
        seg = (tid - adders) % nseg_out;
        g = (tid - adders) / nseg_out;
    }
    const size_t id = (g * nseg_out + seg) * comps_out + comp;
#else
    const size_t id = tid;
    const size_t comp = id % comps_out, seg = (id / comps_out) % nseg_out, g = id / (comps_out * nseg_out);
#endif
    Xyzz29<P> r, h;
    bool r_id, h_id;
    if (FIRST) {
        const Xyzz<P> hi = buckets[g * B + 2 * seg + 1];
        xyzz29_from_xyzz<P>(hi, h, h_id);
        if (comp == 0) {
            const Xyzz<P> lo = buckets[g * B + 2 * seg];
            xyzz29_from_xyzz<P>(lo, r, r_id);
            level_add<P>(r, r_id, h, h_id);
        } else {
            r = h;
            r_id = h_id;
        }
    } else {
        const Plane29<P>* lo = in + ((g * (nseg_out * 2) + 2 * seg) * comps_in);
        const Plane29<P>* hi = lo + comps_in;
        if (comp <= (size_t)k) {
            plane_load<P>(lo + comp, r, r_id);
            plane_load<P>(hi + comp, h, h_id);
            level_add<P>(r, r_id, h, h_id);
        } else {
            plane_load<P>(hi, r, r_id);
        }
    }
    if (LAST) {
        out_host[id] = xyzz29_to_xyzz<P>(r, r_id);
    } else {
        Plane29<P> o;
        o.p = r;
        o.id = r_id;
        o.pad[0] = o.pad[1] = o.pad[2] = 0;
        out[id] = o;
    }
}

template <class P, bool FIRST>
__global__ LURK_REDUCE_BOUNDS void msm_planes29_quad_kernel(const Xyzz<P>* __restrict__ buckets, const Plane29<P>* __restrict__ in,
                                                                           Plane29<P>* __restrict__ out, int k, int G, uint32_t B) {
    __builtin_amdgcn_s_setprio(3);
    const size_t nseg_out = (size_t)B >> (k + 2);
    const size_t ci = (size_t)k + 1, co = ci + 2;
    const size_t tid = (size_t)blockIdx.x * REDUCE_BLOCK + threadIdx.x;
    const size_t heavy = (size_t)G * nseg_out * ci;
    if (tid >= heavy + (size_t)G * nseg_out) return;
    size_t comp, seg, g;
    const bool light = tid >= heavy;
    if (!light) {
        comp = tid % ci;
        seg = (tid / ci) % nseg_out;
        g = tid / (ci * nseg_out);
    } else {
        comp = 0;
        seg = (tid - heavy) % nseg_out;
        g = (tid - heavy) / nseg_out;
    }
    auto load = [&](int q, Xyzz29<P>& v, bool& id) {
        if (FIRST) {
            const Xyzz<P> b = buckets[g * B + 4 * seg + q];
            xyzz29_from_xyzz<P>(b, v, id);
        } else {
            plane_load<P>(in + ((g * (nseg_out * 4) + 4 * seg + q) * ci + comp), v, id);
        }
    };
    auto store = [&](size_t c_out, const Xyzz29<P>& v, bool id) {
        Plane29<P> o;
        o.p = v;
        o.id = id;
        o.pad[0] = o.pad[1] = o.pad[2] = 0;
        out[(g * nseg_out + seg) * co + c_out] = o;
    };
    Xyzz29<P> r, h;
    bool r_id, h_id;
    if (light) {
        load(1, r, r_id);
        load(3, h, h_id);
        level_add<P>(r, r_id, h, h_id);
        store(ci, r, r_id);
        return;
    }
    load(2, r, r_id);
    load(3, h, h_id);
    level_add<P>(r, r_id, h, h_id);
    if (comp == 0) store(ci + 1, r, r_id);
    load(0, h, h_id);
    level_add<P>(r, r_id, h, h_id);
    load(1, h, h_id);
    level_add<P>(r, r_id, h, h_id);
    store(comp, r, r_id);
}

template <class P, bool LAST>
__global__ LURK_REDUCE_BOUNDS void msm_planes29_wave_kernel(const Plane29<P>* __restrict__ in, Plane29<P>* __restrict__ out,
                                                                           Xyzz<P>* __restrict__ out_host, int K, int LOG, int G, uint32_t nseg_in) {
    __builtin_amdgcn_s_setprio(3);
    const size_t comps_in = (size_t)K + 1, comps_out = comps_in + LOG;
    const uint32_t lane = threadIdx.x & 63;
    const size_t wave = ((size_t)blockIdx.x * REDUCE_BLOCK + threadIdx.x) >> 6;
    const size_t chunks = ((size_t)nseg_in + 63) / 64;
    if (wave >= (size_t)G * comps_out * chunks) return;
    const size_t chunk = wave % chunks, comp = (wave / chunks) % comps_out, g = wave / (chunks * comps_out);
    const size_t seg = chunk * 64 + lane;
    Xyzz29<P> r;
    bool r_id = true;
#pragma unroll
    for (int i = 0; i < 9; i++) r.x.l[i] = r.y.l[i] = r.zz.l[i] = r.zzz.l[i] = 0;
    if (seg < nseg_in) {
        const Plane29<P>* src = in + (g * nseg_in + seg) * comps_in;
        if (comp < comps_in) plane_load<P>(src + comp, r, r_id);
        else if ((seg >> (comp - comps_in)) & 1) plane_load<P>(src, r, r_id);
    }
    for (int t = 0; t < LOG; t++) {
        const int m = 1 << t;
        Xyzz29<P> h;
#pragma unroll
        for (int i = 0; i < 9; i++) {
            h.x.l[i] = (uint32_t)__shfl_xor((int)r.x.l[i], m);
            h.y.l[i] = (uint32_t)__shfl_xor((int)r.y.l[i], m);
            h.zz.l[i] = (uint32_t)__shfl_xor((int)r.zz.l[i], m);
            h.zzz.l[i] = (uint32_t)__shfl_xor((int)r.zzz.l[i], m);
        }
        const bool h_id = __shfl_xor((int)r_id, m) != 0;
        xyzz29_add<P>(r, r_id, h, h_id);
    }
    if ((lane & ((1u << LOG) - 1u)) != 0 || seg >= nseg_in) return;
    const size_t nseg_out = (size_t)nseg_in >> LOG;
    const size_t id = (g * nseg_out + (seg >> LOG)) * comps_out + comp;
    if (LAST) {
        out_host[id] = xyzz29_to_xyzz<P>(r, r_id);
    } else {
        Plane29<P> o;
        o.p = r;
        o.id = r_id;
        o.pad[0] = o.pad[1] = o.pad[2] = 0;
        out[id] = o;
    }
}

#ifndef LURK_MSM_BN254_TU
size_t msm_reduce_plane_bytes(size_t nb) { return nb * 160; }
#endif

static bool reduce_wave_levels() {
    static const bool on = [] { const char* v = getenv("LURK_MSM_REDUCE_WAVE"); return !v || atoi(v) != 0; }();
    return on;
}

static bool reduce_quad_levels() {
    static const bool on = [] { const char* v = getenv("LURK_MSM_REDUCE_QUAD"); return !v || atoi(v) != 0; }();
    return on;
}

template <class P>
void msm_launch_reduce(const Xyzz<P>* buckets, void* planes_a, void* planes_b, int c, int G, uint32_t B, Xyzz<P>* out_host, hipStream_t s) {
    static_assert(sizeof(Plane29<P>) == 160, "plane record");
    Plane29<P>* bufs[2] = {(Plane29<P>*)planes_a, (Plane29<P>*)planes_b};
    int K = c - 1;
    if (reduce_wave_levels() && c >= 3 && B == (1u << (c - 1))) {
        K = c - 1 > 12 ? c - 1 - 12 : 0;
        if (K < 1) K = 1;
        const size_t cap = (size_t)num_cus() * 4 * 2;
        auto waves = [&](int k) {
            const int rem = c - 1 - k, log1 = rem > 6 ? rem - rem / 2 : rem;
            return (size_t)G * ((((size_t)B >> k) + 63) / 64) * (size_t)(k + 1 + log1);
        };
        while (K < c - 1 && waves(K) > cap) K++;
    }
    const Plane29<P>* src = bufs[1];
    Plane29<P>* dst = bufs[0];
    auto swap = [&] {
        Plane29<P>* t = dst;
        dst = const_cast<Plane29<P>*>(src);
        src = t;
    };
    int k = 0;
    while (k < K) {
        if (reduce_quad_levels() && k + 2 <= K && k + 2 <= c - 2) {
            const size_t threads = (size_t)G * ((size_t)B >> (k + 2)) * (k + 2);
            const dim3 grid(div_up(threads, REDUCE_BLOCK)), block(REDUCE_BLOCK);
            if (k == 0) hipLaunchKernelGGL((msm_planes29_quad_kernel<P, true>), grid, block, 0, s, buckets, src, dst, k, G, B);
            else hipLaunchKernelGGL((msm_planes29_quad_kernel<P, false>), grid, block, 0, s, buckets, src, dst, k, G, B);
            k += 2;
        } else {
            const size_t threads = (size_t)G * ((size_t)B >> (k + 1)) * (k + 2);
            const dim3 grid(div_up(threads, REDUCE_BLOCK)), block(REDUCE_BLOCK);
            const bool last = k == c - 2;
            if (k == 0 && last) hipLaunchKernelGGL((msm_planes29_kernel<P, true, true>), grid, block, 0, s, buckets, src, dst, out_host, k, G, B);
            else if (k == 0) hipLaunchKernelGGL((msm_planes29_kernel<P, true, false>), grid, block, 0, s, buckets, src, dst, out_host, k, G, B);
            else if (last) hipLaunchKernelGGL((msm_planes29_kernel<P, false, true>), grid, block, 0, s, buckets, src, dst, out_host, k, G, B);
            else hipLaunchKernelGGL((msm_planes29_kernel<P, false, false>), grid, block, 0, s, buckets, src, dst, out_host, k, G, B);
            k += 1;
        }
        swap();
    }
    while (k < c - 1) {
        const int rem = c - 1 - k, log = rem > 6 ? rem - rem / 2 : rem;
        const uint32_t nseg_in = B >> k;
        const size_t nwaves = (size_t)G * (((size_t)nseg_in + 63) / 64) * (size_t)(k + 1 + log);
        const dim3 grid(div_up(nwaves * 64, REDUCE_BLOCK)), block(REDUCE_BLOCK);
        if (k + log == c - 1) hipLaunchKernelGGL((msm_planes29_wave_kernel<P, true>), grid, block, 0, s, src, dst, out_host, k, log, G, nseg_in);
        else hipLaunchKernelGGL((msm_planes29_wave_kernel<P, false>), grid, block, 0, s, src, dst, out_host, k, log, G, nseg_in);
        swap();
        k += log;
    }
    LURK_HIP_CHECK(hipGetLastError());
}
#ifdef LURK_MSM_BN254_TU
template void msm_launch_reduce<Bn254Fq>(const Xyzz<Bn254Fq>*, void*, void*, int, int, uint32_t, Xyzz<Bn254Fq>*, hipStream_t);
template void msm_launch_reduce<Bn254Fr>(const Xyzz<Bn254Fr>*, void*, void*, int, int, uint32_t, Xyzz<Bn254Fr>*, hipStream_t);
#else
template void msm_launch_reduce<PallasFp>(const Xyzz<PallasFp>*, void*, void*, int, int, uint32_t, Xyzz<PallasFp>*, hipStream_t);
template void msm_launch_reduce<PallasFq>(const Xyzz<PallasFq>*, void*, void*, int, int, uint32_t, Xyzz<PallasFq>*, hipStream_t);
#endif

}
```

lurk_beta_amd/csrc/msm_sort.hpp:

```cpp
#pragma once
#include <cstddef>
#include <cstdint>

#include <hip/hip_runtime.h>

namespace lurk {

constexpr int MSM_P_MIN = 2048;
constexpr int MSM_P_MAX = 8192;
#ifndef LURK_SORT_BLOCK
#define LURK_SORT_BLOCK 1024
#endif
constexpr int MSM_SORT_BLOCK = LURK_SORT_BLOCK;
constexpr int MSM_P_PER_MAX = MSM_P_MAX / MSM_SORT_BLOCK;
constexpr int MSM_NB1 = 256 * (1024 / MSM_SORT_BLOCK);
constexpr int MSM_S = 64;
constexpr int MSM_S_MIN = 8;
constexpr size_t MSM_TASK_TARGET = 131072;
constexpr size_t MSM_LDS_BYTES = 160 * 1024;
constexpr int MSM_LB_MAX = 8;

struct MsmShape {
    int c, W, G;
    uint32_t B, NB;
    int P;
    int tile;
    int LB;
    int NG;
    size_t n, stride;
    int S;
    int sel;
    int low_prio;
};

inline size_t msm_scatter1_lds(int P, int W, int tile) { return (size_t)(3 * P + 32) * 4 + (size_t)W * tile * 8; }
inline size_t msm_part2_cap(int LB) { return (MSM_LDS_BYTES - (((size_t)1 << LB) + 32) * 4) / 4; }
inline size_t msm_inter_bytes(size_t entries) { return entries * 5 + 16; }

MsmShape msm_make_shape(int c, bool precomputed, size_t npoints, size_t n, int sel);

struct MsmSortBufs {
    void* inter;
    uint32_t* sorted;
    uint32_t* block_hist;
    uint32_t* part_cnt;
    uint32_t* part_start;
    uint32_t* cnt;
    uint32_t* bucket_start;
    void* canon;
    uint32_t* zero[3];
    int zero_n[3];
};
template <class SF>
void msm_launch_sort(const MsmShape& sh, const void* d_scalars, int is_mont, const MsmSortBufs& b, hipStream_t s);
void msm_launch_sort_canonical(const MsmShape& sh, const void* d_scalars, const MsmSortBufs& b, hipStream_t s);

}
```

lurk_beta_amd/csrc/msm_stages.hpp:

```cpp
#pragma once
#include "common.hpp"
#include "msm_core.cuh"

namespace lurk {

constexpr int MSM_SLOTS = LURK_MSM_SLOTS;
constexpr int MSM_ACC_BLOCK = 256;
constexpr int MSM_FIN_SMALL = 16;
constexpr size_t MSM_SMALL_MAX_POINTS = (size_t)1 << 16;

void msm_launch_plan_tasks(const uint32_t* cnt, const uint32_t* bucket_start, uint32_t* task_start, uint32_t* group_tasks, uint32_t* group_task_base,
                           int NG, uint2* task_info, uint32_t* len_hist, uint32_t* order, size_t nt, uint32_t S, int low, hipStream_t s);

template <class P>
void msm_launch_accumulate(const uint32_t* sorted, const Affine<P>* table, const uint2* task_info, const uint32_t* order,
                           const uint32_t* group_task_base, int NG, Xyzz<P>* partials, size_t nt, hipStream_t s);
template <class P>
void msm_launch_accumulate_persistent(const uint32_t* sorted, const Affine<P>* table, const uint2* task_info, const uint32_t* order,
                                      const uint32_t* group_task_base, int NG, Xyzz<P>* partials, uint32_t* cursor, hipStream_t s, unsigned wgs_per_cu = 0);

int msm_bucket_direct_lanes(size_t NB, size_t entries);
template <class P>
void msm_launch_bucket_direct(const uint32_t* sorted, const Affine<P>* table, const uint32_t* bucket_start, const uint32_t* cnt, uint32_t NB, size_t entries,
                              Xyzz<P>* buckets, uint32_t* big_list, uint32_t* big_count, hipStream_t s);

template <class P>
void msm_launch_finalize(const Xyzz<P>* partials, const uint32_t* cnt, const uint32_t* task_start, const uint32_t* group_task_base, uint32_t NB,
                         Xyzz<P>* buckets, uint32_t* big_list, uint32_t* big_count, uint32_t S, hipStream_t s);
template <class P>
void msm_launch_big_buckets(const Xyzz<P>* partials, const uint32_t* cnt, const uint32_t* task_start, const uint32_t* group_task_base, Xyzz<P>* buckets,
                            const uint32_t* big_list, const uint32_t* big_count, uint32_t S, hipStream_t s);

size_t msm_reduce_plane_bytes(size_t nb);
template <class P>
void msm_launch_reduce(const Xyzz<P>* buckets, void* planes_a, void* planes_b, int c, int G, uint32_t B, Xyzz<P>* out_host, hipStream_t s);

size_t msm_precompute_scratch_bytes(size_t n, int W);
template <class P>
void msm_launch_precompute(const Affine<P>* bases, size_t n, Affine<P>* table, int c, int W, void* scratch, hipStream_t s);

int msm_small_window_bits(size_t n);
size_t msm_small_table_entries(size_t n, int c);
unsigned msm_small_groups(size_t n, int c);
unsigned msm_small_out_points(unsigned groups);
size_t msm_small_group_bytes();
size_t msm_small_scratch_bytes();
template <class P>
void msm_small_build_table(const Affine<P>* wbases, size_t n, int c, Affine<P>* table, hipStream_t s);
template <class P, class SF>
void msm_small_launch(const void* d_scalars, size_t n, int is_mont, const Affine<P>* table, int c, void* group_pts, uint32_t* counter, Xyzz<P>* out,
                      hipStream_t s);

}
```

Measured before the change: 1087.

## Store bucket partials and finals as 29-bit plane records in one unified buffer

```diff
diff --git a/lurk_beta_amd/csrc/curve29.cuh b/lurk_beta_amd/csrc/curve29.cuh
--- a/lurk_beta_amd/csrc/curve29.cuh
+++ b/lurk_beta_amd/csrc/curve29.cuh
@@ -305,6 +305,82 @@
     }
     return xyzz29_to_xyzz<P>(acc, acc_id);
 }
+
+template <class P>
+struct Plane29 {
+    Xyzz29<P> p;
+    uint32_t id, pad[3];
+};
+template <class P>
+LURK_HD void plane_load(const Plane29<P>* __restrict__ src, Xyzz29<P>& v, bool& id) {
+    const Plane29<P> r = *src;
+    v = r.p;
+    id = r.id != 0;
+}
+template <class P>
+LURK_HD void plane_store(Plane29<P>* __restrict__ dst, const Xyzz29<P>& v, bool id) {
+    if (!id) {
+        F29_ASSERT_LIMBS(v.x, 29, "record x"); F29_ASSERT_TOP(v.x, 27, "record x");
+        F29_ASSERT_LIMBS(v.y, 29, "record y"); F29_ASSERT_TOP(v.y, 27, "record y");
+        F29_ASSERT_LIMBS(v.zz, 29, "record zz"); F29_ASSERT_TOP(v.zz, 27, "record zz");
+        F29_ASSERT_LIMBS(v.zzz, 29, "record zzz"); F29_ASSERT_TOP(v.zzz, 27, "record zzz");
+    }
+    Plane29<P> o;
+    o.p = v;
+    o.id = id;
+    o.pad[0] = o.pad[1] = o.pad[2] = 0;
+    *dst = o;
+}
+template <class P>
+LURK_HD void plane_store_identity(Plane29<P>* __restrict__ dst) {
+    Xyzz29<P> z;
+    z.x = z.y = z.zz = z.zzz = f29_zero<P>();
+    plane_store<P>(dst, z, true);
+}
+template <class P>
+LURK_HD void plane_sum(const Plane29<P>* recs, uint32_t nt, Xyzz29<P>& acc, bool& acc_id) {
+    plane_load<P>(recs, acc, acc_id);
+    for (uint32_t i = 1; i < nt; i++) {
+        Xyzz29<P> q;
+        bool q_id;
+        plane_load<P>(recs + i, q, q_id);
+        xyzz29_add<P>(acc, acc_id, q, q_id);
+    }
+}
+
+template <class P>
+LURK_HD bool plane_finalize_bucket(Plane29<P>* records, uint32_t NB, size_t key, uint32_t nt, uint32_t first, uint32_t fin_small) {
+    if (nt == 1) return false;
+    if (nt == 0) {
+        plane_store_identity<P>(records + key);
+        return false;
+    }
+    if (nt > fin_small) return true;
+    Xyzz29<P> acc;
+    bool acc_id;
+    plane_sum<P>(records + NB + first, nt, acc, acc_id);
+    plane_store<P>(records + key, acc, acc_id);
+    return false;
+}
+
+#if defined(__HIPCC__)
+template <class P, int BLOCK>
+__device__ __forceinline__ void block_tree_sum29(Xyzz29<P>& acc, bool& acc_id, Plane29<P>* sh) {
+    const int t = threadIdx.x;
+    plane_store<P>(sh + t, acc, acc_id);
+    __syncthreads();
+    for (int stride = BLOCK / 2; stride >= 1; stride >>= 1) {
+        if (t < stride) {
+            Xyzz29<P> q;
+            bool q_id;
+            plane_load<P>(sh + t + stride, q, q_id);
+            xyzz29_add<P>(acc, acc_id, q, q_id);
+            plane_store<P>(sh + t, acc, acc_id);
+        }
+        __syncthreads();
+    }
+}
+#endif
 
 typedef uint32_t Rec16 __attribute__((vector_size(16), may_alias));
 struct Rec64 {
diff --git a/lurk_beta_amd/csrc/msm.hip b/lurk_beta_amd/csrc/msm.hip
--- a/lurk_beta_amd/csrc/msm.hip
+++ b/lurk_beta_amd/csrc/msm.hip
@@ -26,7 +26,8 @@
     struct Work {
         std::mutex mu;
         DevBuf inter, sorted, block_hist, part_cnt, part_start, cnt, bucket_start, task_start, group_tasks, group_task_base, task_info,
-            task_order, len_hist, partials, buckets, big_list, big_count, planes_a, planes_b, canon, small_counter;
+            task_dest,
+            task_order, len_hist, records, partials , big_list, big_count, planes_a, planes_b, canon, small_counter;
         Xyzz<P>* host_pts = nullptr;
         size_t ws_n = 0, ws_entries = 0, ws_nt = 0;
         uint32_t ws_NB = 0;
@@ -57,14 +58,14 @@
         const Work& wk;
         static uint32_t* u32(const DevBuf& b) { return (uint32_t*)b.p; }
         uint32_t *sorted = u32(wk.sorted), *cnt = u32(wk.cnt), *bucket_start = u32(wk.bucket_start), *task_start = u32(wk.task_start),
-                 *group_tasks = u32(wk.group_tasks), *group_task_base = u32(wk.group_task_base), *task_order = u32(wk.task_order),
+                 *group_tasks = u32(wk.group_tasks), *group_task_base = u32(wk.group_task_base), *task_dest = u32(wk.task_dest), *task_order = u32(wk.task_order),
                  *len_hist = u32(wk.len_hist), *big_list = u32(wk.big_list), *big_count = u32(wk.big_count), *cursor = u32(wk.cursor);
         uint2* task_info = (uint2*)wk.task_info.p;
-        Xyzz<P>*partials = (Xyzz<P>*)wk.partials.p, *buckets = (Xyzz<P>*)wk.buckets.p;
+        Plane29<P>* records = (Plane29<P>*)wk.records.p;
         void *planes_a = wk.planes_a.p, *planes_b = wk.planes_b.p;
         MsmSortBufs sort_bufs() const {
             return MsmSortBufs{wk.inter.p, sorted, u32(wk.block_hist), u32(wk.part_cnt), u32(wk.part_start), cnt, bucket_start, wk.canon.p,
-                               {big_count, len_hist, cursor}, {1, 2 * (MSM_S + 1), MSM_PLACEMENT_BASE + 512}};
+                               {big_count, len_hist, cursor}, {1, 2 * (MSM_S_MAX + 1), MSM_PLACEMENT_BASE + 512}};
         }
     };
     Work work[MSM_SLOTS];
@@ -287,10 +288,10 @@
         wk.group_tasks.ensure(64 * 4);
         wk.group_task_base.ensure(64 * 4);
         wk.task_info.ensure(nt * sizeof(uint2));
+        wk.task_dest.ensure(nt * 4);
         wk.task_order.ensure(nt * 4);
-        wk.len_hist.ensure(2 * (MSM_S + 1) * 4);
-        wk.partials.ensure(nt * sizeof(Xyzz<P>));
-        wk.buckets.ensure((size_t)sh.NB * sizeof(Xyzz<P>));
+        wk.len_hist.ensure(2 * (MSM_S_MAX + 1) * 4);
+        wk.records.ensure(((size_t)(sh.NB > wk.ws_NB ? sh.NB : wk.ws_NB) + (nt > wk.ws_nt ? nt : wk.ws_nt)) * MSM_RECORD_BYTES);
         wk.big_list.ensure((size_t)sh.NB * 4);
         wk.big_count.ensure(16);
         wk.cursor.ensure(4 * (MSM_PLACEMENT_BASE + 512));
@@ -329,6 +330,7 @@
         MsmShape sh = shape(n, L.sel);
         const int low = L.plan.low_prio ? 1 : 0;
         sh.low_prio = low;
+        if (form == MsmAccForm::PERSISTENT_ACC_STREAM && sh.S == MSM_S) sh.S = msm_tuning().persist_s;
         ensure_workspace(wk, sh);
         if (is_mont) wk.canon.ensure(n * 32);
         const WorkView v{wk};
@@ -339,8 +341,8 @@
         }
         if (!direct) {
             ProfScope ps("msm_tasks", s);
-            msm_launch_plan_tasks(v.cnt, v.bucket_start, v.task_start, v.group_tasks, v.group_task_base, sh.NG, v.task_info, v.len_hist, v.task_order, nt,
-                                  (uint32_t)sh.S, low, s);
+            msm_launch_plan_tasks(v.cnt, v.bucket_start, v.task_start, v.group_tasks, v.group_task_base, sh.NG, sh.NB, v.task_info, v.task_dest, v.len_hist,
+                                  v.task_order, nt, (uint32_t)sh.S, low, s);
         }
         if (L.before_accumulate) (*L.before_accumulate)();
         if (wk.planned) LURK_HIP_CHECK(hipEventRecord(wk.planned, s));
@@ -348,14 +350,15 @@
         switch (form) {
         case MsmAccForm::DIRECT: {
             ProfScope ps("msm_accumulate_direct", s);
-            msm_launch_bucket_direct<P>(v.sorted, table, v.bucket_start, v.cnt, sh.NB, (size_t)sh.W * sh.n, v.buckets, v.big_list, v.big_count, s);
+            msm_launch_bucket_direct<P>(v.sorted, table, v.bucket_start, v.cnt, sh.NB, (size_t)sh.W * sh.n, v.records, v.big_list, v.big_count, s);
             break;
         }
         case MsmAccForm::PERSISTENT_SLOT_STREAM: {
             wk.placement_valid = true;
             {
                 ProfScope ps("msm_accumulate_persistent", s);
-                msm_launch_accumulate_persistent<P>(v.sorted, table, v.task_info, v.task_order, v.group_task_base, sh.NG, v.partials, v.cursor, s, L.plan.wgs_per_cu);
+                msm_launch_accumulate_persistent<P>(v.sorted, table, v.task_info, v.task_order, v.task_dest, v.group_task_base, sh.NG, v.records, v.cursor, s,
+                                                    L.plan.wgs_per_cu);
             }
             LURK_HIP_CHECK(hipEventRecord(wk.accumulated, s));
             break;
@@ -376,7 +379,8 @@
             }
             {
                 ProfScope ps("msm_accumulate_persistent", L.acc_stream);
-                msm_launch_accumulate_persistent<P>(v.sorted, table, v.task_info, v.task_order, v.group_task_base, sh.NG, v.partials, v.cursor, L.acc_stream);
+                msm_launch_accumulate_persistent<P>(v.sorted, table, v.task_info, v.task_order, v.task_dest, v.group_task_base, sh.NG, v.records, v.cursor,
+                                                    L.acc_stream);
             }
             LURK_HIP_CHECK(hipEventRecord(wk.accumulated, L.acc_stream));
             LURK_HIP_CHECK(hipStreamWaitEvent(s, wk.accumulated, 0));
@@ -385,7 +389,7 @@
         case MsmAccForm::PLAIN: {
             {
                 ProfScope ps("msm_accumulate", s);
-                msm_launch_accumulate<P>(v.sorted, table, v.task_info, v.task_order, v.group_task_base, sh.NG, v.partials, nt, s);
+                msm_launch_accumulate<P>(v.sorted, table, v.task_info, v.task_order, v.task_dest, v.group_task_base, sh.NG, v.records, nt, s);
             }
             if (wk.accumulated) LURK_HIP_CHECK(hipEventRecord(wk.accumulated, s));
             break;
@@ -393,12 +397,12 @@
         }
         if (!direct) {
             ProfScope ps("msm_finalize", s);
-            msm_launch_finalize<P>(v.partials, v.cnt, v.task_start, v.group_task_base, sh.NB, v.buckets, v.big_list, v.big_count, (uint32_t)sh.S, s);
-            msm_launch_big_buckets<P>(v.partials, v.cnt, v.task_start, v.group_task_base, v.buckets, v.big_list, v.big_count, (uint32_t)sh.S, s);
+            msm_launch_finalize<P>(v.records, v.cnt, v.task_start, v.group_task_base, sh.NB, v.big_list, v.big_count, (uint32_t)sh.S, s);
+            msm_launch_big_buckets<P>(v.records, v.cnt, v.task_start, v.group_task_base, sh.NB, v.big_list, v.big_count, (uint32_t)sh.S, s);
         }
         {
             ProfScope ps("msm_reduce", s);
-            msm_launch_reduce<P>(v.buckets, v.planes_a, v.planes_b, sh.c, sh.G, sh.B, wk.host_pts, s);
+            msm_launch_reduce<P>(v.records, v.planes_a, v.planes_b, sh.c, sh.G, sh.B, wk.host_pts, s);
         }
         LURK_HIP_CHECK(hipGetLastError());
     }
diff --git a/lurk_beta_amd/csrc/msm_acc.hip b/lurk_beta_amd/csrc/msm_acc.hip
--- a/lurk_beta_amd/csrc/msm_acc.hip
+++ b/lurk_beta_amd/csrc/msm_acc.hip
@@ -12,25 +12,26 @@
 template <class P>
 __global__ __launch_bounds__(MSM_ACC_BLOCK) void msm_accumulate_kernel(const uint32_t* __restrict__ sorted, const Affine<P>* __restrict__ table,
                                                                          const uint2* __restrict__ task_info, const uint32_t* __restrict__ order,
+                                                                         const uint32_t* __restrict__ task_dest,
                                                                          const uint32_t* __restrict__ group_task_base, int NG,
-                                                                         Xyzz<P>* __restrict__ partials) {
+                                                                         Plane29<P>* __restrict__ records) {
 #if !defined(LURK_ACC_NO_SETPRIO)
     __builtin_amdgcn_s_setprio(1);
 #endif
     uint32_t i = blockIdx.x * MSM_ACC_BLOCK + threadIdx.x;
     if (i >= group_task_base[NG]) return;
-    msm_accumulate_task<P>(i, sorted, table, task_info, order, partials);
+    msm_accumulate_task<P>(i, sorted, table, task_info, order, task_dest, records);
 }
 
 template <class P>
-void msm_launch_accumulate(const uint32_t* sorted, const Affine<P>* table, const uint2* task_info, const uint32_t* order,
-                           const uint32_t* group_task_base, int NG, Xyzz<P>* partials, size_t nt, hipStream_t s) {
-    hipLaunchKernelGGL((msm_accumulate_kernel<P>), dim3(div_up(nt, MSM_ACC_BLOCK)), dim3(MSM_ACC_BLOCK), 0, s, sorted, table, task_info, order,
-                       group_task_base, NG, partials);
+void msm_launch_accumulate(const uint32_t* sorted, const Affine<P>* table, const uint2* task_info, const uint32_t* order, const uint32_t* task_dest,
+                           const uint32_t* group_task_base, int NG, Plane29<P>* records, size_t nt, hipStream_t s) {
+    hipLaunchKernelGGL((msm_accumulate_kernel<P>), dim3(div_up(nt, MSM_ACC_BLOCK)), dim3(MSM_ACC_BLOCK), 0, s, sorted, table, task_info, order, task_dest,
+                       group_task_base, NG, records);
 }
-#define LURK_ACC_INSTANTIATE(P)                                                                                                             \
-    template void msm_launch_accumulate<P>(const uint32_t*, const Affine<P>*, const uint2*, const uint32_t*, const uint32_t*, int, Xyzz<P>*, \
-                                           size_t, hipStream_t);
+#define LURK_ACC_INSTANTIATE(P)                                                                                                                  \
+    template void msm_launch_accumulate<P>(const uint32_t*, const Affine<P>*, const uint2*, const uint32_t*, const uint32_t*, const uint32_t*, int, \
+                                           Plane29<P>*, size_t, hipStream_t);
 #ifdef LURK_MSM_BN254_TU
 LURK_ACC_INSTANTIATE(Bn254Fq)
 LURK_ACC_INSTANTIATE(Bn254Fr)
diff --git a/lurk_beta_amd/csrc/msm_acc_persistent.hip b/lurk_beta_amd/csrc/msm_acc_persistent.hip
--- a/lurk_beta_amd/csrc/msm_acc_persistent.hip
+++ b/lurk_beta_amd/csrc/msm_acc_persistent.hip
@@ -23,8 +23,9 @@
 __global__ __launch_bounds__(MSM_ACC_BLOCK, LURK_PERSIST_MIN_BLOCKS) __attribute__((amdgpu_num_vgpr(LURK_PERSIST_VGPR_BUDGET / 2))) void msm_accumulate_persistent_kernel(const uint32_t* __restrict__ sorted, const Affine<P>* __restrict__ table,
                                                                                     const uint2* __restrict__ task_info,
                                                                                     const uint32_t* __restrict__ order,
+                                                                                    const uint32_t* __restrict__ task_dest,
                                                                                     const uint32_t* __restrict__ group_task_base, int NG,
-                                                                                    Xyzz<P>* __restrict__ partials, uint32_t* __restrict__ cursor) {
+                                                                                    Plane29<P>* __restrict__ records, uint32_t* __restrict__ cursor) {
     const uint32_t ntasks = group_task_base[NG];
     const uint32_t lane = threadIdx.x & 63u;
     if (threadIdx.x == 0) atomicAdd(&cursor[MSM_PLACEMENT_BASE + msm_cu_index()], 1u);
@@ -33,25 +34,25 @@
         if (lane == 0) base = atomicAdd(cursor, 64u);
         base = __builtin_amdgcn_readfirstlane(base);
         if (base >= ntasks) break;
-        if (base + lane < ntasks) msm_accumulate_task<P, PIPELINED>(base + lane, sorted, table, task_info, order, partials);
+        if (base + lane < ntasks) msm_accumulate_task<P, PIPELINED>(base + lane, sorted, table, task_info, order, task_dest, records);
     }
 }
 
 template <class P>
-void msm_launch_accumulate_persistent(const uint32_t* sorted, const Affine<P>* table, const uint2* task_info, const uint32_t* order,
-                                      const uint32_t* group_task_base, int NG, Xyzz<P>* partials, uint32_t* cursor, hipStream_t s, unsigned wgs_per_cu) {
+void msm_launch_accumulate_persistent(const uint32_t* sorted, const Affine<P>* table, const uint2* task_info, const uint32_t* order, const uint32_t* task_dest,
+                                      const uint32_t* group_task_base, int NG, Plane29<P>* records, uint32_t* cursor, hipStream_t s, unsigned wgs_per_cu) {
     static const unsigned wgs = [] { const char* e = getenv("LURK_MSM_PERSIST_WGS"); int v = e ? atoi(e) : 1; return (unsigned)(v < 1 ? 1 : v > 4 ? 4 : v); }();
     const unsigned waves = wgs_per_cu ? wgs_per_cu : wgs;
     if (waves == 1)
         hipLaunchKernelGGL((msm_accumulate_persistent_kernel<P, true>), dim3((unsigned)num_cus()), dim3(MSM_ACC_BLOCK), 0, s, sorted, table, task_info, order,
-                           group_task_base, NG, partials, cursor);
+                           task_dest, group_task_base, NG, records, cursor);
     else
         hipLaunchKernelGGL((msm_accumulate_persistent_kernel<P, false>), dim3((unsigned)num_cus() * waves), dim3(MSM_ACC_BLOCK), 0, s, sorted, table, task_info, order,
-                           group_task_base, NG, partials, cursor);
+                           task_dest, group_task_base, NG, records, cursor);
 }
 #define LURK_ACC_PERSISTENT_INSTANTIATE(P)                                                                                                    \
-    template void msm_launch_accumulate_persistent<P>(const uint32_t*, const Affine<P>*, const uint2*, const uint32_t*, const uint32_t*, int, \
-                                                      Xyzz<P>*, uint32_t*, hipStream_t, unsigned);
+    template void msm_launch_accumulate_persistent<P>(const uint32_t*, const Affine<P>*, const uint2*, const uint32_t*, const uint32_t*, const uint32_t*, int, \
+                                                      Plane29<P>*, uint32_t*, hipStream_t, unsigned);
 #ifdef LURK_MSM_BN254_TU
 LURK_ACC_PERSISTENT_INSTANTIATE(Bn254Fq)
 LURK_ACC_PERSISTENT_INSTANTIATE(Bn254Fr)
diff --git a/lurk_beta_amd/csrc/msm_acc_task.cuh b/lurk_beta_amd/csrc/msm_acc_task.cuh
--- a/lurk_beta_amd/csrc/msm_acc_task.cuh
+++ b/lurk_beta_amd/csrc/msm_acc_task.cuh
@@ -16,14 +16,17 @@
 template <class P, bool PIPELINED = false>
 __device__ LURK_ACC_TASK_ATTR void msm_accumulate_task(uint32_t i, const uint32_t* __restrict__ sorted, const Affine<P>* __restrict__ table,
                                                     const uint2* __restrict__ task_info, const uint32_t* __restrict__ order,
-                                                    Xyzz<P>* __restrict__ partials) {
+                                                    const uint32_t* __restrict__ task_dest, Plane29<P>* __restrict__ records) {
     uint32_t t = order[i];
     uint2 ti = task_info[t];
+    Xyzz29<P> acc;
+    bool acc_id;
 #if LURK_ACC_RADIX29
-    partials[t] = msm_task_accumulate29<P, PIPELINED>(sorted, ti.x, ti.y, table);
+    msm_task_accumulate29_raw<P, PIPELINED>(sorted, ti.x, ti.y, table, acc, acc_id);
 #else
-    partials[t] = msm_task_accumulate<P>(sorted, ti.x, ti.y, table);
+    xyzz29_from_xyzz<P>(msm_task_accumulate<P>(sorted, ti.x, ti.y, table), acc, acc_id);
 #endif
+    plane_store<P>(records + task_dest[t], acc, acc_id);
 }
 
 }
diff --git a/lurk_beta_amd/csrc/msm_bucket_direct.hip b/lurk_beta_amd/csrc/msm_bucket_direct.hip
--- a/lurk_beta_amd/csrc/msm_bucket_direct.hip
+++ b/lurk_beta_amd/csrc/msm_bucket_direct.hip
@@ -11,7 +11,7 @@
 template <class P, int L>
 __global__ __launch_bounds__(DIRECT_BLOCK) void msm_bucket_direct_kernel(const uint32_t* __restrict__ sorted, const Affine<P>* __restrict__ table,
                                                                            const uint32_t* __restrict__ bucket_start, const uint32_t* __restrict__ cnt,
-                                                                           uint32_t NB, Xyzz<P>* __restrict__ buckets, uint32_t* __restrict__ big_list,
+                                                                           uint32_t NB, Plane29<P>* __restrict__ buckets, uint32_t* __restrict__ big_list,
                                                                            uint32_t* __restrict__ big_count) {
     __builtin_amdgcn_s_setprio(1);
     const size_t lane = (size_t)blockIdx.x * DIRECT_BLOCK + threadIdx.x;
@@ -47,39 +47,29 @@
         o_id = __shfl_xor((int)acc_id, off) != 0;
         xyzz29_add<P>(acc, acc_id, o, o_id);
     }
-    if (live && !big && sub == 0) buckets[key] = xyzz29_to_xyzz<P>(acc, acc_id);
+    if (live && !big && sub == 0) plane_store<P>(buckets + key, acc, acc_id);
 }
 
 template <class P>
 __global__ __launch_bounds__(DIRECT_BLOCK) void msm_bucket_direct_big_kernel(const uint32_t* __restrict__ sorted, const Affine<P>* __restrict__ table,
                                                                                const uint32_t* __restrict__ bucket_start, const uint32_t* __restrict__ cnt,
-                                                                               Xyzz<P>* __restrict__ buckets, const uint32_t* __restrict__ big_list,
+                                                                               Plane29<P>* __restrict__ buckets, const uint32_t* __restrict__ big_list,
                                                                                const uint32_t* __restrict__ big_count) {
     __builtin_amdgcn_s_setprio(1);
     extern __shared__ uint4 lds_raw[];
-    Xyzz<P>* sh = reinterpret_cast<Xyzz<P>*>(lds_raw);
+    Plane29<P>* sh = reinterpret_cast<Plane29<P>*>(lds_raw);
     const uint32_t nbig = *big_count;
     for (uint32_t i = blockIdx.x; i < nbig; i += gridDim.x) {
         const uint32_t key = big_list[i], n = cnt[key], start = bucket_start[key];
-        Xyzz29<P> a29;
-        a29.x = a29.y = a29.zz = a29.zzz = f29_zero<P>();
-        bool a_id = true;
+        Xyzz29<P> acc;
+        acc.x = acc.y = acc.zz = acc.zzz = f29_zero<P>();
+        bool acc_id = true;
         for (uint32_t j = threadIdx.x; j < n; j += DIRECT_BLOCK) {
             const uint32_t e = sorted[start + j];
-            xyzz29_madd<P>(a29, a_id, table[e & 0x7fffffffu], (e & 0x80000000u) != 0);
+            xyzz29_madd<P>(acc, acc_id, table[e & 0x7fffffffu], (e & 0x80000000u) != 0);
         }
-        Xyzz<P> acc = xyzz29_to_xyzz<P>(a29, a_id);
-        const int t = threadIdx.x;
-        sh[t] = acc;
-        __syncthreads();
-        for (int stride = DIRECT_BLOCK / 2; stride >= 1; stride >>= 1) {
-            if (t < stride) {
-                xyzz_add<P>(acc, sh[t + stride]);
-                sh[t] = acc;
-            }
-            __syncthreads();
-        }
-        if (t == 0) buckets[key] = acc;
+        block_tree_sum29<P, DIRECT_BLOCK>(acc, acc_id, sh);
+        if (threadIdx.x == 0) plane_store<P>(buckets + key, acc, acc_id);
         __syncthreads();
     }
 }
@@ -94,17 +84,17 @@
 
 template <class P>
 void msm_launch_bucket_direct(const uint32_t* sorted, const Affine<P>* table, const uint32_t* bucket_start, const uint32_t* cnt, uint32_t NB, size_t entries,
-                              Xyzz<P>* buckets, uint32_t* big_list, uint32_t* big_count, hipStream_t s) {
+                              Plane29<P>* buckets, uint32_t* big_list, uint32_t* big_count, hipStream_t s) {
     const int L = msm_bucket_direct_lanes(NB, entries);
     const dim3 grid((unsigned)div_up((size_t)NB * L, DIRECT_BLOCK)), block(DIRECT_BLOCK);
     if (L == 1) hipLaunchKernelGGL((msm_bucket_direct_kernel<P, 1>), grid, block, 0, s, sorted, table, bucket_start, cnt, NB, buckets, big_list, big_count);
     else if (L == 2) hipLaunchKernelGGL((msm_bucket_direct_kernel<P, 2>), grid, block, 0, s, sorted, table, bucket_start, cnt, NB, buckets, big_list, big_count);
     else hipLaunchKernelGGL((msm_bucket_direct_kernel<P, 4>), grid, block, 0, s, sorted, table, bucket_start, cnt, NB, buckets, big_list, big_count);
-    hipLaunchKernelGGL((msm_bucket_direct_big_kernel<P>), dim3(128), block, DIRECT_BLOCK * sizeof(Xyzz<P>), s, sorted, table, bucket_start, cnt, buckets, big_list,
+    hipLaunchKernelGGL((msm_bucket_direct_big_kernel<P>), dim3(128), block, DIRECT_BLOCK * sizeof(Plane29<P>), s, sorted, table, bucket_start, cnt, buckets, big_list,
                        big_count);
 }
 #define LURK_DIRECT_INSTANTIATE(P)                                                                                                                      \
-    template void msm_launch_bucket_direct<P>(const uint32_t*, const Affine<P>*, const uint32_t*, const uint32_t*, uint32_t, size_t, Xyzz<P>*, uint32_t*, \
+    template void msm_launch_bucket_direct<P>(const uint32_t*, const Affine<P>*, const uint32_t*, const uint32_t*, uint32_t, size_t, Plane29<P>*, uint32_t*, \
                                               uint32_t*, hipStream_t);
 #ifdef LURK_MSM_BN254_TU
 LURK_DIRECT_INSTANTIATE(Bn254Fq)
diff --git a/lurk_beta_amd/csrc/msm_finalize.hip b/lurk_beta_amd/csrc/msm_finalize.hip
--- a/lurk_beta_amd/csrc/msm_finalize.hip
+++ b/lurk_beta_amd/csrc/msm_finalize.hip
@@ -10,33 +10,64 @@
 #endif
 #define LURK_FINALIZE_BOUNDS __launch_bounds__(256, LURK_FINALIZE_WAVES)
 template <class P>
-__global__ LURK_FINALIZE_BOUNDS void msm_finalize_kernel(const Xyzz<P>* __restrict__ partials, const uint32_t* __restrict__ cnt,
-                                                             const uint32_t* __restrict__ task_start,
-                                                             const uint32_t* __restrict__ group_task_base, uint32_t NB,
-                                                             Xyzz<P>* __restrict__ buckets, uint32_t* __restrict__ big_list,
+__global__ LURK_FINALIZE_BOUNDS void msm_finalize_kernel(Plane29<P>* records, const uint32_t* __restrict__ cnt, const uint32_t* __restrict__ task_start,
+                                                             const uint32_t* __restrict__ group_task_base, uint32_t NB, uint32_t* __restrict__ big_list,
                                                              uint32_t* __restrict__ big_count, uint32_t S) {
     __builtin_amdgcn_s_setprio(3);
     const size_t key = (size_t)blockIdx.x * 256 + threadIdx.x;
     if (key >= NB) return;
-    const uint32_t g = (uint32_t)(key / MSM_GRP), b = (uint32_t)(key % MSM_GRP);
     const uint32_t nt = (cnt[key] + S - 1) / S;
-    const uint32_t first = group_task_base[g] + task_start[(size_t)g * (MSM_GRP + 1) + b];
-    if (nt > MSM_FIN_SMALL) {
-        big_list[atomicAdd(big_count, 1u)] = (uint32_t)key;
-        return;
+    uint32_t first = 0;
+    if (nt >= 2 && nt <= MSM_FIN_SMALL) {
+        const uint32_t g = (uint32_t)(key / MSM_GRP), b = (uint32_t)(key % MSM_GRP);
+        first = group_task_base[g] + task_start[(size_t)g * (MSM_GRP + 1) + b];
     }
-    buckets[key] = xyzz_sum_via29<P>(partials + first, nt);
+    if (plane_finalize_bucket<P>(records, NB, key, nt, first, MSM_FIN_SMALL)) big_list[atomicAdd(big_count, 1u)] = (uint32_t)key;
 }
 
 template <class P>
-void msm_launch_finalize(const Xyzz<P>* partials, const uint32_t* cnt, const uint32_t* task_start, const uint32_t* group_task_base, uint32_t NB,
-                         Xyzz<P>* buckets, uint32_t* big_list, uint32_t* big_count, uint32_t S, hipStream_t s) {
-    hipLaunchKernelGGL((msm_finalize_kernel<P>), dim3(div_up((size_t)NB, 256)), dim3(256), 0, s, partials, cnt, task_start, group_task_base, NB, buckets,
-                       big_list, big_count, S);
+__global__ LURK_FINALIZE_BOUNDS void msm_big_bucket_kernel(Plane29<P>* records, const uint32_t* __restrict__ cnt, const uint32_t* __restrict__ task_start,
+                                                               const uint32_t* __restrict__ group_task_base, uint32_t NB,
+                                                               const uint32_t* __restrict__ big_list, const uint32_t* __restrict__ big_count, uint32_t S) {
+    __builtin_amdgcn_s_setprio(3);
+    extern __shared__ uint4 lds_raw[];
+    Plane29<P>* sh = reinterpret_cast<Plane29<P>*>(lds_raw);
+    const uint32_t nbig = *big_count;
+    for (uint32_t i = blockIdx.x; i < nbig; i += gridDim.x) {
+        const uint32_t key = big_list[i];
+        const uint32_t g = key / MSM_GRP, b = key % MSM_GRP;
+        const uint32_t nt = (cnt[key] + S - 1) / S;
+        const Plane29<P>* tasks = records + NB + (group_task_base[g] + task_start[(size_t)g * (MSM_GRP + 1) + b]);
+        Xyzz29<P> acc, q;
+        acc.x = acc.y = acc.zz = acc.zzz = f29_zero<P>();
+        bool acc_id = true, q_id;
+        for (uint32_t j = threadIdx.x; j < nt; j += 256) {
+            plane_load<P>(tasks + j, q, q_id);
+            xyzz29_add<P>(acc, acc_id, q, q_id);
+        }
+        block_tree_sum29<P, 256>(acc, acc_id, sh);
+        if (threadIdx.x == 0) plane_store<P>(records + key, acc, acc_id);
+        __syncthreads();
+    }
 }
-#define LURK_FINALIZE_INSTANTIATE(P)                                                                                                          \
-    template void msm_launch_finalize<P>(const Xyzz<P>*, const uint32_t*, const uint32_t*, const uint32_t*, uint32_t, Xyzz<P>*, uint32_t*, uint32_t*, \
-                                         uint32_t, hipStream_t);
+
+template <class P>
+void msm_launch_finalize(Plane29<P>* records, const uint32_t* cnt, const uint32_t* task_start, const uint32_t* group_task_base, uint32_t NB,
+                         uint32_t* big_list, uint32_t* big_count, uint32_t S, hipStream_t s) {
+    static_assert(sizeof(Plane29<P>) == MSM_RECORD_BYTES, "the slot's record array is sized by MSM_RECORD_BYTES");
+    hipLaunchKernelGGL((msm_finalize_kernel<P>), dim3(div_up((size_t)NB, 256)), dim3(256), 0, s, records, cnt, task_start, group_task_base, NB, big_list, big_count,
+                       S);
+}
+template <class P>
+void msm_launch_big_buckets(Plane29<P>* records, const uint32_t* cnt, const uint32_t* task_start, const uint32_t* group_task_base, uint32_t NB,
+                            const uint32_t* big_list, const uint32_t* big_count, uint32_t S, hipStream_t s) {
+    hipLaunchKernelGGL((msm_big_bucket_kernel<P>), dim3(128), dim3(256), 256 * sizeof(Plane29<P>), s, records, cnt, task_start, group_task_base, NB, big_list,
+                       big_count, S);
+}
+#define LURK_FINALIZE_INSTANTIATE(P)                                                                                                                      \
+    template void msm_launch_finalize<P>(Plane29<P>*, const uint32_t*, const uint32_t*, const uint32_t*, uint32_t, uint32_t*, uint32_t*, uint32_t, hipStream_t); \
+    template void msm_launch_big_buckets<P>(Plane29<P>*, const uint32_t*, const uint32_t*, const uint32_t*, uint32_t, const uint32_t*, const uint32_t*, uint32_t, \
+                                            hipStream_t);
 #ifdef LURK_MSM_BN254_TU
 LURK_FINALIZE_INSTANTIATE(Bn254Fq)
 LURK_FINALIZE_INSTANTIATE(Bn254Fr)
diff --git a/lurk_beta_amd/csrc/msm_launch_plan.hpp b/lurk_beta_amd/csrc/msm_launch_plan.hpp
--- a/lurk_beta_amd/csrc/msm_launch_plan.hpp
+++ b/lurk_beta_amd/csrc/msm_launch_plan.hpp
@@ -25,6 +25,7 @@
 struct MsmTuning {
     int persistent = 1, max_acc = 2, placement_log = 0, bucket_direct = 1;
     size_t persistent_min = (size_t)24 << 20;
+    int persist_s = 128;
     static MsmTuning from_env() {
         auto geti = [](const char* k, int d) { const char* v = getenv(k); return v ? atoi(v) : d; };
         MsmTuning t;
@@ -33,6 +34,7 @@
         t.max_acc = geti("LURK_MSM_MAX_ACC", 2);
         t.bucket_direct = geti("LURK_MSM_BUCKET_DIRECT", 1);
         t.placement_log = geti("LURK_MSM_PLACEMENT_LOG", 0);
+        t.persist_s = geti("LURK_MSM_PERSIST_S", 128) == 64 ? 64 : 128;
         if (t.max_acc > 2) t.max_acc = 0;
         return t;
     }
diff --git a/lurk_beta_amd/csrc/msm_plan.hip b/lurk_beta_amd/csrc/msm_plan.hip
--- a/lurk_beta_amd/csrc/msm_plan.hip
+++ b/lurk_beta_amd/csrc/msm_plan.hip
@@ -51,7 +51,8 @@
 constexpr int MSM_NG_MAX = 64;
 __global__ __launch_bounds__(256) void msm_tasks_kernel(const uint32_t* __restrict__ cnt, const uint32_t* __restrict__ bucket_start,
                                                           const uint32_t* __restrict__ task_start, const uint32_t* __restrict__ group_tasks,
-                                                          uint32_t* __restrict__ group_task_base_out, int NG, uint2* __restrict__ task_info, uint32_t S, int low) {
+                                                          uint32_t* __restrict__ group_task_base_out, int NG, uint32_t NB, uint2* __restrict__ task_info,
+                                                          uint32_t* __restrict__ task_dest, uint32_t S, int low) {
     msm_set_wave_prio(low);
     __shared__ uint32_t group_task_base[MSM_NG_MAX + 1];
     if (threadIdx.x == 0) {
@@ -77,13 +78,14 @@
     uint32_t first = bucket_start[key] + part * S;
     uint32_t end = bucket_start[key] + cnt[key];
     task_info[t] = make_uint2(first, first + S < end ? first + S : end);
+    task_dest[t] = cnt[key] <= S ? (uint32_t)key : NB + t;
 }
 
 __global__ __launch_bounds__(1024) void msm_len_hist_kernel(const uint2* __restrict__ task_info, const uint32_t* __restrict__ group_task_base,
                                                               int NG, uint32_t* __restrict__ len_hist, uint32_t S, int low) {
     msm_set_wave_prio(low);
-    __shared__ uint32_t sh[MSM_S + 1];
-    if (threadIdx.x <= MSM_S) sh[threadIdx.x] = 0;
+    __shared__ uint32_t sh[MSM_S_MAX + 1];
+    if (threadIdx.x <= MSM_S_MAX) sh[threadIdx.x] = 0;
     __syncthreads();
     const uint32_t ntasks = group_task_base[NG];
     for (uint32_t base = blockIdx.x * 8192u; base < ntasks; base += gridDim.x * 8192u) {
@@ -100,14 +102,14 @@
         }
     }
     __syncthreads();
-    if (threadIdx.x <= MSM_S && sh[threadIdx.x]) atomicAdd(&len_hist[threadIdx.x], sh[threadIdx.x]);
+    if (threadIdx.x <= MSM_S_MAX && sh[threadIdx.x]) atomicAdd(&len_hist[threadIdx.x], sh[threadIdx.x]);
 }
 __global__ __launch_bounds__(1024) void msm_len_scatter_kernel(const uint2* __restrict__ task_info,
                                                                  const uint32_t* __restrict__ group_task_base, int NG,
                                                                  const uint32_t* __restrict__ len_hist, uint32_t* __restrict__ len_cursor,
                                                                  uint32_t* __restrict__ order, uint32_t S, int low) {
     msm_set_wave_prio(low);
-    __shared__ uint32_t sh_cnt[MSM_S + 1], sh_base[MSM_S + 1], sh_class[MSM_S + 1];
+    __shared__ uint32_t sh_cnt[MSM_S_MAX + 1], sh_base[MSM_S_MAX + 1], sh_class[MSM_S_MAX + 1];
     if (threadIdx.x == 0) {
         uint32_t run = 0;
         for (int l = (int)S; l >= 0; l--) {
@@ -118,7 +120,7 @@
     __syncthreads();
     const uint32_t ntasks = group_task_base[NG];
     for (uint32_t base = blockIdx.x * 1024u; base < ntasks; base += gridDim.x * 1024u) {
-        if (threadIdx.x <= MSM_S) sh_cnt[threadIdx.x] = 0;
+        if (threadIdx.x <= MSM_S_MAX) sh_cnt[threadIdx.x] = 0;
         __syncthreads();
         uint32_t t = base + threadIdx.x;
         uint32_t len = 0, rank = 0;
@@ -137,7 +139,7 @@
             rank = atomicAdd(&sh_cnt[len], 1u);
         }
         __syncthreads();
-        if (threadIdx.x <= MSM_S && sh_cnt[threadIdx.x]) sh_base[threadIdx.x] = sh_class[threadIdx.x] + atomicAdd(&len_cursor[threadIdx.x], sh_cnt[threadIdx.x]);
+        if (threadIdx.x <= MSM_S_MAX && sh_cnt[threadIdx.x]) sh_base[threadIdx.x] = sh_class[threadIdx.x] + atomicAdd(&len_cursor[threadIdx.x], sh_cnt[threadIdx.x]);
         __syncthreads();
         if (len != 0) order[sh_base[len] + rank] = t;
         __syncthreads();
@@ -145,62 +147,13 @@
 }
 
 void msm_launch_plan_tasks(const uint32_t* cnt, const uint32_t* bucket_start, uint32_t* task_start, uint32_t* group_tasks, uint32_t* group_task_base,
-                           int NG, uint2* task_info, uint32_t* len_hist, uint32_t* order, size_t nt, uint32_t S, int low, hipStream_t s) {
+                           int NG, uint32_t NB, uint2* task_info, uint32_t* task_dest, uint32_t* len_hist, uint32_t* order, size_t nt, uint32_t S, int low,
+                           hipStream_t s) {
     hipLaunchKernelGGL(msm_taskscan_kernel, dim3(NG), dim3(1024), 0, s, cnt, task_start, group_tasks, S, low);
-    hipLaunchKernelGGL(msm_tasks_kernel, dim3(div_up(nt, 256)), dim3(256), 0, s, cnt, bucket_start, task_start, group_tasks, group_task_base, NG, task_info, S,
-                       low);
+    hipLaunchKernelGGL(msm_tasks_kernel, dim3(div_up(nt, 256)), dim3(256), 0, s, cnt, bucket_start, task_start, group_tasks, group_task_base, NG, NB, task_info,
+                       task_dest, S, low);
     hipLaunchKernelGGL(msm_len_hist_kernel, dim3(256), dim3(1024), 0, s, task_info, group_task_base, NG, len_hist, S, low);
-    hipLaunchKernelGGL(msm_len_scatter_kernel, dim3(512), dim3(1024), 0, s, task_info, group_task_base, NG, len_hist, len_hist + MSM_S + 1, order, S, low);
+    hipLaunchKernelGGL(msm_len_scatter_kernel, dim3(512), dim3(1024), 0, s, task_info, group_task_base, NG, len_hist, len_hist + MSM_S_MAX + 1, order, S, low);
 }
 
-template <class P, int BLOCK>
-__device__ void block_tree_sum(Xyzz<P>& acc, Xyzz<P>* sh) {
-    const int t = threadIdx.x;
-    sh[t] = acc;
-    __syncthreads();
-    for (int stride = BLOCK / 2; stride >= 1; stride >>= 1) {
-        if (t < stride) {
-            xyzz_add<P>(acc, sh[t + stride]);
-            sh[t] = acc;
-        }
-        __syncthreads();
-    }
 }
-
-template <class P>
-__global__ __launch_bounds__(256) void msm_big_bucket_kernel(const Xyzz<P>* __restrict__ partials, const uint32_t* __restrict__ cnt,
-                                                               const uint32_t* __restrict__ task_start,
-                                                               const uint32_t* __restrict__ group_task_base, Xyzz<P>* __restrict__ buckets,
-                                                               const uint32_t* __restrict__ big_list, const uint32_t* __restrict__ big_count, uint32_t S) {
-    msm_set_wave_prio(0);
-    extern __shared__ uint4 lds_raw[];
-    Xyzz<P>* sh = reinterpret_cast<Xyzz<P>*>(lds_raw);
-    const uint32_t nbig = *big_count;
-    for (uint32_t i = blockIdx.x; i < nbig; i += gridDim.x) {
-        uint32_t key = big_list[i];
-        uint32_t g = key / MSM_GRP, b = key % MSM_GRP;
-        uint32_t nt = (cnt[key] + S - 1) / S;
-        uint32_t first = group_task_base[g] + task_start[(size_t)g * (MSM_GRP + 1) + b];
-        Xyzz<P> acc = xyzz_identity<P>();
-        for (uint32_t j = threadIdx.x; j < nt; j += 256) xyzz_add<P>(acc, partials[first + j]);
-        block_tree_sum<P, 256>(acc, sh);
-        if (threadIdx.x == 0) buckets[key] = acc;
-        __syncthreads();
-    }
-}
-
-template <class P>
-void msm_launch_big_buckets(const Xyzz<P>* partials, const uint32_t* cnt, const uint32_t* task_start, const uint32_t* group_task_base, Xyzz<P>* buckets,
-                            const uint32_t* big_list, const uint32_t* big_count, uint32_t S, hipStream_t s) {
-    hipLaunchKernelGGL((msm_big_bucket_kernel<P>), dim3(128), dim3(256), 256 * sizeof(Xyzz<P>), s, partials, cnt, task_start, group_task_base, buckets, big_list,
-                       big_count, S);
-}
-#define LURK_BIG_BUCKETS_INSTANTIATE(P)                                                                                                                   \
-    template void msm_launch_big_buckets<P>(const Xyzz<P>*, const uint32_t*, const uint32_t*, const uint32_t*, Xyzz<P>*, const uint32_t*, const uint32_t*, \
-                                            uint32_t, hipStream_t);
-LURK_BIG_BUCKETS_INSTANTIATE(PallasFp)
-LURK_BIG_BUCKETS_INSTANTIATE(PallasFq)
-LURK_BIG_BUCKETS_INSTANTIATE(Bn254Fq)
-LURK_BIG_BUCKETS_INSTANTIATE(Bn254Fr)
-
-}
diff --git a/lurk_beta_amd/csrc/msm_reduce.hip b/lurk_beta_amd/csrc/msm_reduce.hip
--- a/lurk_beta_amd/csrc/msm_reduce.hip
+++ b/lurk_beta_amd/csrc/msm_reduce.hip
@@ -27,21 +27,9 @@
 
 constexpr int REDUCE_BLOCK = 256;
 
-template <class P>
-struct Plane29 {
-    Xyzz29<P> p;
-    uint32_t id, pad[3];
-};
-
-template <class P>
-__device__ __forceinline__ void plane_load(const Plane29<P>* __restrict__ src, Xyzz29<P>& v, bool& id) {
-    const Plane29<P> r = *src;
-    v = r.p;
-    id = r.id != 0;
-}
 
 template <class P, bool FIRST, bool LAST>
-__global__ LURK_REDUCE_BOUNDS void msm_planes29_kernel(const Xyzz<P>* __restrict__ buckets, const Plane29<P>* __restrict__ in,
+__global__ LURK_REDUCE_BOUNDS void msm_planes29_kernel(const Plane29<P>* __restrict__ buckets, const Plane29<P>* __restrict__ in,
                                                                       Plane29<P>* __restrict__ out, Xyzz<P>* __restrict__ out_host, int k, int G, uint32_t B) {
     __builtin_amdgcn_s_setprio(3);
     const size_t nseg_out = (size_t)B >> (k + 1);
@@ -68,11 +56,9 @@
     Xyzz29<P> r, h;
     bool r_id, h_id;
     if (FIRST) {
-        const Xyzz<P> hi = buckets[g * B + 2 * seg + 1];
-        xyzz29_from_xyzz<P>(hi, h, h_id);
+        plane_load<P>(buckets + (g * B + 2 * seg + 1), h, h_id);
         if (comp == 0) {
-            const Xyzz<P> lo = buckets[g * B + 2 * seg];
-            xyzz29_from_xyzz<P>(lo, r, r_id);
+            plane_load<P>(buckets + (g * B + 2 * seg), r, r_id);
             level_add<P>(r, r_id, h, h_id);
         } else {
             r = h;
@@ -92,16 +78,12 @@
     if (LAST) {
         out_host[id] = xyzz29_to_xyzz<P>(r, r_id);
     } else {
-        Plane29<P> o;
-        o.p = r;
-        o.id = r_id;
-        o.pad[0] = o.pad[1] = o.pad[2] = 0;
-        out[id] = o;
+        plane_store<P>(out + id, r, r_id);
     }
 }
 
 template <class P, bool FIRST>
-__global__ LURK_REDUCE_BOUNDS void msm_planes29_quad_kernel(const Xyzz<P>* __restrict__ buckets, const Plane29<P>* __restrict__ in,
+__global__ LURK_REDUCE_BOUNDS void msm_planes29_quad_kernel(const Plane29<P>* __restrict__ buckets, const Plane29<P>* __restrict__ in,
                                                                            Plane29<P>* __restrict__ out, int k, int G, uint32_t B) {
     __builtin_amdgcn_s_setprio(3);
     const size_t nseg_out = (size_t)B >> (k + 2);
@@ -122,18 +104,13 @@
     }
     auto load = [&](int q, Xyzz29<P>& v, bool& id) {
         if (FIRST) {
-            const Xyzz<P> b = buckets[g * B + 4 * seg + q];
-            xyzz29_from_xyzz<P>(b, v, id);
+            plane_load<P>(buckets + (g * B + 4 * seg + q), v, id);
         } else {
             plane_load<P>(in + ((g * (nseg_out * 4) + 4 * seg + q) * ci + comp), v, id);
         }
     };
     auto store = [&](size_t c_out, const Xyzz29<P>& v, bool id) {
-        Plane29<P> o;
-        o.p = v;
-        o.id = id;
-        o.pad[0] = o.pad[1] = o.pad[2] = 0;
-        out[(g * nseg_out + seg) * co + c_out] = o;
+        plane_store<P>(out + ((g * nseg_out + seg) * co + c_out), v, id);
     };
     Xyzz29<P> r, h;
     bool r_id, h_id;
@@ -194,11 +171,7 @@
     if (LAST) {
         out_host[id] = xyzz29_to_xyzz<P>(r, r_id);
     } else {
-        Plane29<P> o;
-        o.p = r;
-        o.id = r_id;
-        o.pad[0] = o.pad[1] = o.pad[2] = 0;
-        out[id] = o;
+        plane_store<P>(out + id, r, r_id);
     }
 }
 
@@ -217,7 +190,7 @@
 }
 
 template <class P>
-void msm_launch_reduce(const Xyzz<P>* buckets, void* planes_a, void* planes_b, int c, int G, uint32_t B, Xyzz<P>* out_host, hipStream_t s) {
+void msm_launch_reduce(const Plane29<P>* buckets, void* planes_a, void* planes_b, int c, int G, uint32_t B, Xyzz<P>* out_host, hipStream_t s) {
     static_assert(sizeof(Plane29<P>) == 160, "plane record");
     Plane29<P>* bufs[2] = {(Plane29<P>*)planes_a, (Plane29<P>*)planes_b};
     int K = c - 1;
@@ -271,11 +244,11 @@
     LURK_HIP_CHECK(hipGetLastError());
 }
 #ifdef LURK_MSM_BN254_TU
-template void msm_launch_reduce<Bn254Fq>(const Xyzz<Bn254Fq>*, void*, void*, int, int, uint32_t, Xyzz<Bn254Fq>*, hipStream_t);
-template void msm_launch_reduce<Bn254Fr>(const Xyzz<Bn254Fr>*, void*, void*, int, int, uint32_t, Xyzz<Bn254Fr>*, hipStream_t);
-#else
-template void msm_launch_reduce<PallasFp>(const Xyzz<PallasFp>*, void*, void*, int, int, uint32_t, Xyzz<PallasFp>*, hipStream_t);
-template void msm_launch_reduce<PallasFq>(const Xyzz<PallasFq>*, void*, void*, int, int, uint32_t, Xyzz<PallasFq>*, hipStream_t);
-#endif
-
-}
+template void msm_launch_reduce<Bn254Fq>(const Plane29<Bn254Fq>*, void*, void*, int, int, uint32_t, Xyzz<Bn254Fq>*, hipStream_t);
+template void msm_launch_reduce<Bn254Fr>(const Plane29<Bn254Fr>*, void*, void*, int, int, uint32_t, Xyzz<Bn254Fr>*, hipStream_t);
+#else
+template void msm_launch_reduce<PallasFp>(const Plane29<PallasFp>*, void*, void*, int, int, uint32_t, Xyzz<PallasFp>*, hipStream_t);
+template void msm_launch_reduce<PallasFq>(const Plane29<PallasFq>*, void*, void*, int, int, uint32_t, Xyzz<PallasFq>*, hipStream_t);
+#endif
+
+}
diff --git a/lurk_beta_amd/csrc/msm_sort.hpp b/lurk_beta_amd/csrc/msm_sort.hpp
--- a/lurk_beta_amd/csrc/msm_sort.hpp
+++ b/lurk_beta_amd/csrc/msm_sort.hpp
@@ -16,6 +16,7 @@
 constexpr int MSM_NB1 = 256 * (1024 / MSM_SORT_BLOCK);
 constexpr int MSM_S = 64;
 constexpr int MSM_S_MIN = 8;
+constexpr int MSM_S_MAX = 128;
 constexpr size_t MSM_TASK_TARGET = 131072;
 constexpr size_t MSM_LDS_BYTES = 160 * 1024;
 constexpr int MSM_LB_MAX = 8;
diff --git a/lurk_beta_amd/csrc/msm_stages.hpp b/lurk_beta_amd/csrc/msm_stages.hpp
--- a/lurk_beta_amd/csrc/msm_stages.hpp
+++ b/lurk_beta_amd/csrc/msm_stages.hpp
@@ -9,31 +9,36 @@
 constexpr int MSM_FIN_SMALL = 16;
 constexpr size_t MSM_SMALL_MAX_POINTS = (size_t)1 << 16;
 
+template <class P>
+struct Plane29;
+constexpr size_t MSM_RECORD_BYTES = 160;
+
 void msm_launch_plan_tasks(const uint32_t* cnt, const uint32_t* bucket_start, uint32_t* task_start, uint32_t* group_tasks, uint32_t* group_task_base,
-                           int NG, uint2* task_info, uint32_t* len_hist, uint32_t* order, size_t nt, uint32_t S, int low, hipStream_t s);
+                           int NG, uint32_t NB, uint2* task_info, uint32_t* task_dest, uint32_t* len_hist, uint32_t* order, size_t nt, uint32_t S, int low,
+                           hipStream_t s);
 
 template <class P>
-void msm_launch_accumulate(const uint32_t* sorted, const Affine<P>* table, const uint2* task_info, const uint32_t* order,
-                           const uint32_t* group_task_base, int NG, Xyzz<P>* partials, size_t nt, hipStream_t s);
+void msm_launch_accumulate(const uint32_t* sorted, const Affine<P>* table, const uint2* task_info, const uint32_t* order, const uint32_t* task_dest,
+                           const uint32_t* group_task_base, int NG, Plane29<P>* records, size_t nt, hipStream_t s);
 template <class P>
-void msm_launch_accumulate_persistent(const uint32_t* sorted, const Affine<P>* table, const uint2* task_info, const uint32_t* order,
-                                      const uint32_t* group_task_base, int NG, Xyzz<P>* partials, uint32_t* cursor, hipStream_t s, unsigned wgs_per_cu = 0);
+void msm_launch_accumulate_persistent(const uint32_t* sorted, const Affine<P>* table, const uint2* task_info, const uint32_t* order, const uint32_t* task_dest,
+                                      const uint32_t* group_task_base, int NG, Plane29<P>* records, uint32_t* cursor, hipStream_t s, unsigned wgs_per_cu = 0);
 
 int msm_bucket_direct_lanes(size_t NB, size_t entries);
 template <class P>
 void msm_launch_bucket_direct(const uint32_t* sorted, const Affine<P>* table, const uint32_t* bucket_start, const uint32_t* cnt, uint32_t NB, size_t entries,
-                              Xyzz<P>* buckets, uint32_t* big_list, uint32_t* big_count, hipStream_t s);
+                              Plane29<P>* records, uint32_t* big_list, uint32_t* big_count, hipStream_t s);
 
 template <class P>
-void msm_launch_finalize(const Xyzz<P>* partials, const uint32_t* cnt, const uint32_t* task_start, const uint32_t* group_task_base, uint32_t NB,
-                         Xyzz<P>* buckets, uint32_t* big_list, uint32_t* big_count, uint32_t S, hipStream_t s);
+void msm_launch_finalize(Plane29<P>* records, const uint32_t* cnt, const uint32_t* task_start, const uint32_t* group_task_base, uint32_t NB,
+                         uint32_t* big_list, uint32_t* big_count, uint32_t S, hipStream_t s);
 template <class P>
-void msm_launch_big_buckets(const Xyzz<P>* partials, const uint32_t* cnt, const uint32_t* task_start, const uint32_t* group_task_base, Xyzz<P>* buckets,
+void msm_launch_big_buckets(Plane29<P>* records, const uint32_t* cnt, const uint32_t* task_start, const uint32_t* group_task_base, uint32_t NB,
                             const uint32_t* big_list, const uint32_t* big_count, uint32_t S, hipStream_t s);
 
 size_t msm_reduce_plane_bytes(size_t nb);
 template <class P>
-void msm_launch_reduce(const Xyzz<P>* buckets, void* planes_a, void* planes_b, int c, int G, uint32_t B, Xyzz<P>* out_host, hipStream_t s);
+void msm_launch_reduce(const Plane29<P>* buckets, void* planes_a, void* planes_b, int c, int G, uint32_t B, Xyzz<P>* out_host, hipStream_t s);
 
 size_t msm_precompute_scratch_bytes(size_t n, int W);
 template <class P>
```

After: 1102, median of 6. 1.01x the previous value.
